# AndrewBoessen/3DGS

Measured on AMD Instinct MI355X. Metric: fwd+bwd iterations/s (one view per GPU), 1e6 gaussians @1920x1080, SH deg 3, higher is better.
Workload: dtype f32; 1 GPU; BASELINE configs[2]: synthetic 1000000 gaussians, 1920x1080, SH deg 3, forward+backward; parallelism=single GPU, exchange=none, backend=none, M=1000000, S=3499903, num_pairs=22157704, scene_seed=15717

## Files before the change

3dgs_amd/_lib.py:

```python
import ctypes
import os
import subprocess

_HERE = os.path.dirname(os.path.abspath(__file__))
_CSRC = os.path.join(_HERE, "csrc")
LIB_PATH = os.path.join(_HERE, "libgsplat_hip.so")
_lib = None


class GsplatError(RuntimeError):
    def __init__(self, code, text):
        super().__init__(f"gsplat error {code}: {text}")
        self.code = code


def build(force=False):
    import fcntl
    srcs = [os.path.join(_CSRC, f) for f in os.listdir(_CSRC) if f.endswith((".hip", ".h")) or f == "Makefile"]
    srcs.append(os.path.join(_CSRC, "host", "gs_dataset.cpp"))
    srcs.append(os.path.join(_HERE, "..", "include", "gsplat_hip.h"))

    def stale():
        return force or not os.path.exists(LIB_PATH) or any(
            os.path.getmtime(s) > os.path.getmtime(LIB_PATH) for s in srcs)
# ... 154 lines not shown
    "gsplat_gather_rows": (_I, [_I, _I, _P, _P, _P, _P]),
    "gsplat_sample_by_weight": (_I, [_P, _I, _I, ctypes.c_ulonglong, _P, _P, _P]),
    "gsplat_mcmc_relocate": (_I, [_I, _P, _P, _P, _F, _P]),
    "gsplat_mcmc_add_noise": (_I, [_I, _P, _P, _P, _P, _F, ctypes.c_ulonglong, _P]),
    "gsplat_mcmc_regularize": (_I, [_I, _P, _P, _P, _F, _F, _P, _P, _P]),
    "gsplat_compact_masked_array": (_I, [_P, _P, _I, _I, _P, ctypes.POINTER(_I), _P]),
    "gsplat_scatter_masked_array": (_I, [_P, _P, _I, _I, _P, _P]),
    "gsplat_context_create": (_I, [ctypes.POINTER(_P), _I, _I, _I]),
    "gsplat_context_destroy": (_I, [_P]),
    "gsplat_context_bytes": (_S, [_P]),
    "gsplat_rasterize_image": (_I, [_P, ctypes.POINTER(Gaussians), ctypes.POINTER(Camera),
                                    ctypes.POINTER(RasterConfig), _F, _I, ctypes.POINTER(ForwardView), _P]),
    "gsplat_backward_pass": (_I, [_P, ctypes.POINTER(Gaussians), ctypes.POINTER(Camera), _P, _F, _I,
                                  ctypes.POINTER(Gradients), _P]),
    "gsplat_backward_gaussians_adam": (_I, [_P, ctypes.POINTER(Gaussians), ctypes.POINTER(Camera), _I,
                                            ctypes.POINTER(AdamFused), ctypes.POINTER(Gradients), _P]),
    "gsplat_context_set_render_only": (_I, [_P, _I]),
    "gsplat_context_set_lean_forward": (_I, [_P, _I]),
    "gsplat_context_set_depth": (_I, [_P, _I]),
    "gsplat_context_depth_map": (_I, [_P, ctypes.POINTER(_P)]),
    "gsplat_backward_render_depth": (_I, [_P, _P, _P, _P, _F, _P, _P, _P, _P]),
    "gsplat_backward_pass_depth": (_I, [_P, ctypes.POINTER(Gaussians), ctypes.POINTER(Camera), _P, _P, _P, _F, _I,
                                        ctypes.POINTER(Gradients), _P]),
    "gsplat_context_set_depth_mode": (_I, [_P, _I, _I]),
    "gsplat_context_depth_moment_map": (_I, [_P, ctypes.POINTER(_P)]),
    "gsplat_backward_render_depth2": (_I, [_P, _P, _P, _P, _P, _F, _P, _P, _P, _P]),
    "gsplat_backward_pass_depth2": (_I, [_P, ctypes.POINTER(Gaussians), ctypes.POINTER(Camera), _P, _P, _P, _P, _F, _I,
                                         ctypes.POINTER(Gradients), _P]),
    "gsplat_distortion_loss": (_I, [_P, _P, _P, _I, _I, _F, _I, _P, _P, _P, _P, _P]),
    "gsplat_depth_prior_loss": (_I, [_P, _P, _I, _I, _F, _I, _P, _P, _P]),
    "gsplat_depth_to_normal": (_I, [_P, _P, _I, _I, _F, _F, _F, _F, _I, _F, _P, _P]),
    "gsplat_depth_to_normal_backward": (_I, [_P, _P, _I, _I, _F, _F, _F, _F, _I, _F, _P, _I, _P, _P, _P]),
    "gsplat_normal_prior_loss": (_I, [_P, _P, _I, _I, _F, _I, _P, _P, _P]),
    "gsplat_normal_smoothness_loss": (_I, [_P, _P, _I, _I, _F, _F, _I, _P, _P, _P]),
    "gsplat_backward_gaussians_camera": (_I, [_P, ctypes.POINTER(Gaussians), ctypes.POINTER(Camera), _I,
                                              ctypes.POINTER(Gradients), _P, _P, _P]),
    "gsplat_backward_pass_camera": (_I, [_P, ctypes.POINTER(Gaussians), ctypes.POINTER(Camera), _P, _P, _P, _F, _I,
                                         ctypes.POINTER(Gradients), _P, _P, _P]),
    "gsplat_context_accumulate_contributions": (_I, [_P, _I, _P, _P, _P, _P]),
    "gsplat_context_render_features": (_I, [_P, _I, _I, _P, _P, _P]),
    "gsplat_context_lift_features": (_I, [_P, _I, _I, _P, _P, _P]),
    "gsplat_context_features_backward": (_I, [_P, _I, _I, _P, _P, _P]),
    "gsplat_feature_ce_loss": (_I, [_P, _P, _I, _I, _I, _F, _I, _P, _P, _P]),
    "gsplat_feature_l1_loss": (_I, [_P, _P, _P, _I, _I, _I, _F, _I, _P, _P, _P]),
    "gsplat_feature_cosine_loss": (_I, [_P, _P, _P, _I, _I, _I, _F, _I, _P, _P, _P]),
    "gsplat_feature_adam_step": (_I, [_P, _I, _I, _P, _P, _P, _P, _F, _F, _F, _F, _F, _F, _P]),
    "gsplat_bilagrid_slice": (_I, [_P, _I, _I, _I, _P, _I, _I, _P, _P]),
    "gsplat_bilagrid_slice_backward": (_I, [_P, _I, _I, _I, _P, _P, _I, _I, _I, _P, _P, _P]),
    "gsplat_bilagrid_tv_loss": (_I, [_P, _I, _I, _I, _F, _I, _P, _P, _P]),
    "gsplat_vq_assign": (_I, [_P, _P, _I, _I, _I, _P, _P, _P]),
    "gsplat_vq_update": (_I, [_P, _P, _P, _I, _I, _I, _P, _P]),
    "gsplat_context_set_absgrad": (_I, [_P, _I]),
    "gsplat_context_set_compact_lists": (_I, [_P, _I]),
    "gsplat_context_absgrad_uv": (_I, [_P, _P, _P]),
    "gsplat_pack_absgrad_norm": (_I, [_P, _I, _P, _P]),
    "gsplat_context_set_antialiased": (_I, [_P, _I]),
    "gsplat_compute_conic_antialiased": (_I, [_P, _P, _P, _F, _F, _F, _F, _F, _I, _P, _P, _P, _P, _P]),
    "gsplat_compute_conic_antialiased_backward": (_I, [_P, _P, _P, _P, _P, _P, _I, _P, _P, _P]),
    "gsplat_compute_filter3d": (_I, [_P, _I, _P, _P, _P, _P, _I, _F, _P, _P]),
    "gsplat_filter3d_apply": (_I, [_P, _P, _P, _I, _P, _P, _P]),
    "gsplat_filter3d_apply_backward": (_I, [_P, _P, _P, _P, _I, _P, _I, _P, _I, _P]),
    "gsplat_context_set_filter3d": (_I, [_P, _P]),
    "gsplat_context_set_preprocess_split": (_I, [_P, _I]),
    "gsplat_context_get_counters": (_I, [_P, ctypes.POINTER(ctypes.c_longlong), _I]),
    "gsplat_context_set_timing": (_I, [_P, _I]),
    "gsplat_context_set_timing_stages": (_I, [_P, ctypes.c_uint]),
    "gsplat_context_get_timing": (_I, [_P, ctypes.POINTER(ctypes.c_double), ctypes.POINTER(ctypes.c_longlong), _I]),
    "gsplat_pack_gradients_global": (_I, [_P, ctypes.POINTER(Gradients), _I, _I, _P, _P]),
    "gsplat_packed_gradient_width": (_I, [_I]),
    "gsplat_factored_gradient_width": (_I, [_I]),
    "gsplat_pack_gradients_factored": (_I, [_P, ctypes.POINTER(Gradients), _I, _I, _I, _P, _P]),
    "gsplat_unpack_gradients_factored": (_I, [_P, _P, _P, _I, _I, _I, _P, _P]),
}


def load():
    global _lib
    if _lib is not None:
        return _lib
    path = os.environ.get("GSPLAT_LIB")
    if not path:
        if os.environ.get("GSPLAT_NO_BUILD") == "1":
            if not os.path.exists(LIB_PATH):
                raise OSError(f"{LIB_PATH} is missing and GSPLAT_NO_BUILD=1 forbids building it")
        else:
            try:
                build()
            except (OSError, subprocess.CalledProcessError) as e:
                if not os.path.exists(LIB_PATH):
                    raise
                import sys
                print(f"[3dgs_amd] WARNING: rebuilding libgsplat_hip.so failed ({e}); loading the EXISTING library, "
                      "which may be older than the sources (the ABI version is checked below)", file=sys.stderr, flush=True)
        path = LIB_PATH
    import torch
    lib = ctypes.CDLL(path)
    for name, (res, args) in SIGNATURES.items():
        fn = getattr(lib, name)
        fn.restype = res
        fn.argtypes = args
    got = lib.gsplat_abi_version()
    if got != ABI_VERSION:
        raise RuntimeError(f"libgsplat_hip.so reports ABI {got}, this binding expects {ABI_VERSION}: stale library")
    built_from, flags = lib.gsplat_source_hash().decode(), lib.gsplat_build_flags().decode()
    if built_from != source_hash() or flags:
        import sys
# ... 22 lines not shown
```

3dgs_amd/csrc/gs_context.h:

```cpp
#pragma once
#include "gs_common.h"
#include "gs_render.h"

namespace gs {

int pre_split_default();
bool pre_join_late();
bool no_tile_order();
bool no_compact_lists();
bool no_segments();
bool no_fwd_segments();
double fwd_segments_gate();

}

struct gsplat_context {
  int max_gaussians = 0, max_width = 0, max_height = 0;
  gs::DeviceBuffer mask, counters, rank, xyz_c_all, uv_all;
  gs::DeviceBuffer c2g, xyz_c, uv, sigma, conic, J, rgb, radius, recs, counts, offsets, grad_rows, hitmask;
  gs::DeviceBuffer keys_a, keys_b, pay_a, pay_b, sorted, temp, bin_table;
  gs::DeviceBuffer blockmasks;
  gs::DeviceBuffer ranges, image, T_px, n_px;
  gs::DeviceBuffer tile_tops, tile_order;
  bool order_ready = false;
  gs::DeviceBuffer ids_c, masks_c, n_c_px, tile_useful;
  bool compact_lists = true;
  bool compact_written = false;
  bool compact_ready = false;
  long long n_compact_backwards = 0;
  gs::DeviceBuffer seg_first, seg_extra, seg_chk;
  gs::DeviceBuffer fseg_first, fseg_blocks, fseg_gran, fseg_part, fseg_stop;
  bool depth = false;
  bool depth_ready = false;
  bool rows_depth = false;
  gs::DeviceBuffer depth_map, seg_chk_d, fseg_part_d;
  bool depth_inverse = false, depth_moment = false;
  bool depth_inverse_ready = false, depth_moment_ready = false;
  gs::DeviceBuffer depth2_map, seg_chk_q, fseg_part_q;
  bool absgrad = false;
  bool rows_abs = false;
  bool antialiased = false;
  bool fwd_antialiased = false;
  const float *filter3d = nullptr;
  const float *fwd_filter3d = nullptr;
  gs::DeviceBuffer f3d_scale, f3d_opacity;
  void *fseg_gran_zeroed = nullptr;
  size_t fseg_gran_zeroed_bytes = 0;
  unsigned int fseg_epoch = 0;
  int fseg_poll_budget = gs::kFwdPollBudget, fseg_thin_layer = gs::kFwdThinLayerDefault;
  double fseg_gate = -1.0;
  unsigned long long n_segmented_forwards = 0;
  gs::Figures fig;
  int seg_cap = 0;
  bool seg_ready = false;
  unsigned long long n_segmented_backwards = 0;
  const unsigned char *last_mask = nullptr;
  int *h_words = nullptr;
  bool dense_route = false;
  int forced_route = 0;
  bool rows_ready = false;
  bool backward_seen = false, rows_zeroed = false;
  bool render_only = false;
  bool lean = false;
  int pre_split = gs::pre_split_default();
  hipStream_t pre_side = nullptr;
  hipEvent_t ev_pre_fork = nullptr, ev_pre_join = nullptr;
  gs::DeviceBuffer chunk_first;
  gs::DeviceBuffer kept;
  gs::DeviceBuffer dir_grad;
  gs::DeviceBuffer cam_rows;
  gs::SortFork fork;
  volatile unsigned long long *h_pub = nullptr;
  unsigned long long *d_pub = nullptr, ticket = 0;
  unsigned long long *pair_counters() const { return counters.as<unsigned long long>(); }
  int *slice_counts() const { return counters.as<int>() + 128; }
  int *fseg_fallbacks() const { return counters.as<int>() + 128 + gs::kBinBlocks; }
  static constexpr int kStages = 8, kSlots = 32;
  unsigned int timing = 0;
  hipEvent_t ev[kSlots][2 * kStages] = {};
  unsigned char pending[kSlots][kStages] = {};
  double stage_ms[kStages] = {};
  long long stage_n[kStages] = {};
  long long fwd_calls = 0;
  long long n_forwards = 0, n_tail_redone = 0, n_compact_walks = 0, n_instance_growths = 0, n_ordered_backwards = 0;
  int slot = 0;
  void mark(int stage, bool stop, hipStream_t st) {
    if (!((timing >> stage) & 1u)) return;
    (void)hipEventRecord(ev[slot][2 * stage + (stop ? 1 : 0)], st);
    if (stop) pending[slot][stage] = 1;
  }
  void harvest(int sl) {
    for (int k = 0; k < kStages; ++k)
      if (pending[sl][k]) {
        float ms = 0.f;
        if (hipEventElapsedTime(&ms, ev[sl][2 * k], ev[sl][2 * k + 1]) == hipSuccess) { stage_ms[k] += ms; stage_n[k] += 1; }
        pending[sl][k] = 0;
      }
  }
  int N = 0, M = 0, l_max = 0, width = 0, height = 0;
  float tan_fovx = 0.f, tan_fovy = 0.f, mh_dist = 0.f;
  size_t S = 0;
  long long last_longest = -1;
  bool have_forward = false;
  bool lists_ready = false;
  enum : unsigned { kCounted = 1u, kOutput = 2u };
  template <class C, class F>
  static void each_buffer(C &c, F &&f) {
    constexpr unsigned W = kCounted, O = kCounted | kOutput;
    f(c.mask, O); f(c.uv_all, O); f(c.xyz_c_all, O); f(c.sigma, O); f(c.conic, O); f(c.J, O); f(c.rgb, O); f(c.radius, O);
    f(c.sorted, O); f(c.ranges, O); f(c.image, O); f(c.T_px, O); f(c.n_px, O);
    f(c.counters, W); f(c.rank, W); f(c.c2g, W); f(c.xyz_c, W); f(c.uv, W); f(c.recs, W); f(c.counts, W); f(c.offsets, W);
    f(c.grad_rows, W); f(c.hitmask, W); f(c.keys_a, W); f(c.keys_b, W); f(c.pay_a, W); f(c.pay_b, W); f(c.temp, W);
    f(c.bin_table, 0u);
    f(c.blockmasks, W); f(c.kept, W); f(c.tile_tops, W); f(c.tile_order, W);
    f(c.ids_c, W); f(c.masks_c, W); f(c.n_c_px, W); f(c.tile_useful, W);
    f(c.seg_first, W); f(c.seg_extra, W); f(c.seg_chk, W);
    f(c.fseg_first, W); f(c.fseg_blocks, W); f(c.fseg_gran, W); f(c.fseg_part, W); f(c.fseg_stop, W);
    f(c.dir_grad, W); f(c.cam_rows, W); f(c.depth_map, W); f(c.seg_chk_d, W); f(c.fseg_part_d, W);
    f(c.depth2_map, W); f(c.seg_chk_q, W); f(c.fseg_part_q, W);
    f(c.f3d_scale, W); f(c.f3d_opacity, W);
    f(c.chunk_first, 0u);
  }
  void forward_outputs(gs::DeviceBuffer *out[13]) {
    int n = 0;
    each_buffer(*this, [&](gs::DeviceBuffer &b, unsigned flags) { if (flags & kOutput) out[n++] = &b; });
  }
  size_t bytes() const {
    size_t total = 0;
    each_buffer(*this, [&](const gs::DeviceBuffer &b, unsigned flags) { if (flags & kCounted) total += b.bytes; });
    return total;
  }
  void release() {
    gs::pool_unwatch(&last_mask);
    last_mask = nullptr;
    each_buffer(*this, [](gs::DeviceBuffer &b, unsigned) { b.release(); });
    fseg_gran_zeroed = nullptr;
    fork.destroy();
    if (pre_side) { (void)hipStreamDestroy(pre_side); pre_side = nullptr; }
    if (ev_pre_fork) { (void)hipEventDestroy(ev_pre_fork); ev_pre_fork = nullptr; }
    if (ev_pre_join) { (void)hipEventDestroy(ev_pre_join); ev_pre_join = nullptr; }
    if (h_words) (void)hipHostFree(h_words);
    h_words = nullptr;
    if (h_pub) { (void)hipHostFree((void *)h_pub); h_pub = nullptr; d_pub = nullptr; }
    for (int a = 0; a < kSlots; ++a)
      for (int b = 0; b < 2 * kStages; ++b)
        if (ev[a][b]) { (void)hipEventDestroy(ev[a][b]); ev[a][b] = nullptr; }
  }
};

namespace gs {
size_t instance_room(const gsplat_context *c);
int reserve_instances(gsplat_context *c, size_t S, int num_tiles, hipStream_t st);
}
```

3dgs_amd/csrc/gs_context.hip:

```cpp
#include <cstdlib>
#include <new>
#include <vector>

#include "gs_context.h"
#include "gs_launch.h"

namespace gs {

static bool env_is(const char *name, char c) { const char *e = getenv(name); return e && e[0] == c; }
static int env_digit(const char *name, int lo, int hi, int otherwise) {
  const char *e = getenv(name);
  return e && e[0] >= '0' + lo && e[0] <= '0' + hi ? e[0] - '0' : otherwise;
}
static double env_number(const char *name, double otherwise) { const char *e = getenv(name); return e && e[0] ? atof(e) : otherwise; }

int pre_split_default() { static const int v = env_digit("GSPLAT_PRE_SPLIT", 0, 2, 0); return v; }
bool pre_join_late() { static const bool v = env_is("GSPLAT_PRE_JOIN", 'l'); return v; }
bool no_tile_order() { static const bool v = env_is("GSPLAT_NO_TILE_ORDER", '1'); return v; }
bool no_compact_lists() { static const bool v = env_is("GSPLAT_NO_COMPACT_LISTS", '1'); return v; }
bool no_segments() { static const bool v = env_is("GSPLAT_NO_SEGMENTS", '1'); return v; }
bool no_fwd_segments() { static const bool v = env_is("GSPLAT_NO_FWD_SEGMENTS", '1'); return v; }
double fwd_segments_gate() { static const double v = env_number("GSPLAT_FWD_SEGMENTS_GATE", 3.0); return v; }

size_t instance_room(const gsplat_context *c) {
  size_t room = c->keys_a.bytes / sizeof(unsigned int);
  room = std::min(room, c->keys_b.bytes / sizeof(unsigned int));
  room = std::min(room, c->pay_a.bytes / sizeof(unsigned long long));
  room = std::min(room, c->pay_b.bytes / sizeof(unsigned long long));
  room = std::min(room, c->sorted.bytes / sizeof(int));
  room = std::min(room, c->blockmasks.bytes / sizeof(unsigned short));
  room = std::min(room, c->ids_c.bytes / sizeof(int));
  room = std::min(room, c->masks_c.bytes / sizeof(unsigned short));
  return room;
}

int reserve_instances(gsplat_context *c, size_t S, int num_tiles, hipStream_t st) {
  int rc;
  const void *pay_before = c->pay_a.ptr, *sorted_before = c->sorted.ptr;
  if ((rc = c->keys_a.reserve((S + 1) * sizeof(unsigned int)))) return rc;
  if ((rc = c->keys_b.reserve((S + 1) * sizeof(unsigned int)))) return rc;
  if ((rc = c->pay_a.reserve((S + 1) * sizeof(unsigned long long)))) return rc;
  if ((rc = c->pay_b.reserve((S + 1) * sizeof(unsigned long long)))) return rc;
  if ((rc = c->sorted.reserve((S + 1) * sizeof(int)))) return rc;
  if (c->pay_a.ptr != pay_before) GS_HIP(hipMemsetAsync(c->pay_a.ptr, 0, c->pay_a.bytes, st));
  if (c->sorted.ptr != sorted_before) GS_HIP(hipMemsetAsync(c->sorted.ptr, 0, c->sorted.bytes, st));
  if ((rc = c->blockmasks.reserve((S + 1) * sizeof(unsigned short)))) return rc;
  if ((rc = c->ids_c.reserve((S + 1) * sizeof(int)))) return rc;
  if ((rc = c->masks_c.reserve((S + 1) * sizeof(unsigned short)))) return rc;
  if ((rc = c->temp.reserve(gs::binning_temp_bytes((size_t)c->max_gaussians, S ? S : 1, num_tiles)))) return rc;
  return GSPLAT_OK;
}

}

extern "C" {

int gsplat_context_create(gsplat_context **out, int max_gaussians, int max_width, int max_height) {
  GS_REQUIRE(out != nullptr, "out is null");
  GS_REQUIRE(max_gaussians > 0 && max_width > 0 && max_height > 0, "capacities must be positive");
  gsplat_context *c = new (std::nothrow) gsplat_context();
  GS_REQUIRE(c != nullptr, "out of host memory");
  c->max_gaussians = max_gaussians; c->max_width = max_width; c->max_height = max_height;
  const size_t N = (size_t)max_gaussians, P = (size_t)max_width * max_height;
  const size_t T = (size_t)((max_width + 15) / 16) * ((max_height + 15) / 16);
  int rc = GSPLAT_OK;
  {
    gs::DeviceBuffer *outs[13];
    c->forward_outputs(outs);
    for (gs::DeviceBuffer *b : outs) b->pooled = true;
  }
  auto R = [&](gs::DeviceBuffer &b, size_t bytes) { if (!rc) rc = b.reserve(bytes); };
  R(c->mask, N + 16); R(c->counters, 512 + gs::kBinBlocks * 4 + 64); R(c->rank, (N + 1) * 4); R(c->xyz_c_all, N * 12); R(c->uv_all, N * 8);
  R(c->c2g, N * 4); R(c->xyz_c, N * 12); R(c->uv, N * 8); R(c->sigma, N * 24); R(c->conic, N * 12); R(c->J, N * 24);
  R(c->rgb, N * 12); R(c->radius, N * 16); R(c->recs, N * 48); R(c->counts, (N + 1) * 4); R(c->offsets, (N + 1) * 4);
  R(c->grad_rows, N * 64); R(c->hitmask, N * 8);
// ... 52 lines not shown
  if (compact_to_global) *compact_to_global = have ? c->c2g.as<int>() : nullptr;
  if (num_gaussians) *num_gaussians = have ? c->N : 0;
  if (num_culled) *num_culled = have ? c->M : 0;
  return GSPLAT_OK;
}

int gsplat_context_detach_forward_outputs(gsplat_context *c) {
  GS_REQUIRE(c != nullptr, "null context");
  GS_REQUIRE(c->n_forwards > 0 && c->mask.ptr != nullptr, "no forward whose outputs could be handed over");
  GS_REQUIRE(!c->lean && !c->render_only, "a lean / render-only forward does not fill all ForwardPassData arrays");
  gs::DeviceBuffer *outs[13];
  c->forward_outputs(outs);
  for (gs::DeviceBuffer *b : outs) (void)b->detach();
  c->have_forward = false;
  c->lists_ready = false;
  c->rows_ready = false;
  return GSPLAT_OK;
}

int gsplat_context_set_depth(gsplat_context *c, int enabled) {
  GS_REQUIRE(c != nullptr, "null context");
  c->depth = enabled != 0;
  c->depth_inverse = c->depth_moment = false;
  return GSPLAT_OK;
}

int gsplat_context_set_depth_mode(gsplat_context *c, int inverse, int moment) {
  GS_REQUIRE(c != nullptr, "null context");
  c->depth = true;
  c->depth_inverse = inverse != 0;
  c->depth_moment = moment != 0;
  return GSPLAT_OK;
}

int gsplat_context_set_antialiased(gsplat_context *c, int enabled) {
  GS_REQUIRE(c != nullptr, "null context");
  c->antialiased = enabled != 0;
  return GSPLAT_OK;
}

int gsplat_context_set_filter3d(gsplat_context *c, const float *filter3d) {
  GS_REQUIRE(c != nullptr, "null context");
  if (filter3d) GS_REQUIRE_DEV(filter3d);
  c->filter3d = filter3d;
  return GSPLAT_OK;
}

int gsplat_context_set_compact_lists(gsplat_context *c, int enabled) {
  GS_REQUIRE(c != nullptr, "null context");
  c->compact_lists = enabled != 0;
  return GSPLAT_OK;
}

int gsplat_context_set_absgrad(gsplat_context *c, int enabled) {
  GS_REQUIRE(c != nullptr, "null context");
  c->absgrad = enabled != 0;
  return GSPLAT_OK;
}

int gsplat_context_accumulate_contributions(gsplat_context *c, int num_gaussians, float *weight_sum, float *weight_max,
                                            int *pixels, void *stream) {
  GS_REQUIRE(c != nullptr, "null context");
  GS_REQUIRE(weight_sum || weight_max || pixels, "no statistic asked for: weight_sum, weight_max and pixels are all NULL");
  GS_REQUIRE(c->lists_ready, "no forward pass recorded in this context");
  GS_REQUIRE(num_gaussians == c->N, "does not match the recorded forward");
  if (weight_sum) GS_REQUIRE_DEV(weight_sum);
  if (weight_max) GS_REQUIRE_DEV(weight_max);
  if (pixels) GS_REQUIRE_DEV(pixels);
  return gs::launch_contributions(c->recs.as<float4>(), c->sorted.as<int>(), c->ranges.as<int>(), c->n_px.as<int>(),
                                  c->c2g.as<int>(), c->width, c->height, weight_sum, weight_max, pixels,
                                  (hipStream_t)stream);
}

int gsplat_context_render_features(gsplat_context *c, int num_gaussians, int channels, const float *features, float *out,
                                   void *stream) {
  GS_REQUIRE(c != nullptr, "null context");
  GS_REQUIRE(c->lists_ready, "no forward pass recorded in this context");
  GS_REQUIRE(num_gaussians == c->N, "does not match the recorded forward");
  GS_REQUIRE(channels >= 1 && channels <= 512, "channels must be 1 .. 512");
  GS_REQUIRE_DEV(features);
  GS_REQUIRE_DEV(out);
  return gs::launch_features_fwd(c->recs.as<float4>(), c->sorted.as<int>(), c->ranges.as<int>(), c->n_px.as<int>(),
                                 c->c2g.as<int>(), c->width, c->height, channels, features, out, (hipStream_t)stream);
}

int gsplat_context_lift_features(gsplat_context *c, int num_gaussians, int channels, const float *map, float *lifted,
                                 void *stream) {
  GS_REQUIRE(c != nullptr, "null context");
  GS_REQUIRE(c->lists_ready, "no forward pass recorded in this context");
  GS_REQUIRE(num_gaussians == c->N, "does not match the recorded forward");
  GS_REQUIRE(channels >= 1 && channels <= 512, "channels must be 1 .. 512");
  GS_REQUIRE_DEV(map);
  GS_REQUIRE_DEV(lifted);
  return gs::launch_features_lift(c->recs.as<float4>(), c->sorted.as<int>(), c->ranges.as<int>(), c->n_px.as<int>(),
                                  c->c2g.as<int>(), c->width, c->height, channels, map, lifted, (hipStream_t)stream);
}

int gsplat_context_features_backward(gsplat_context *c, int num_gaussians, int channels, const float *features,
                                     const float *grad_map, void *stream) {
  GS_REQUIRE(c != nullptr, "null context");
  GS_REQUIRE(c->lists_ready, "no forward pass recorded in this context");
  GS_REQUIRE(c->have_forward && c->rows_ready,
             "gsplat_backward_render has not run for this forward pass: the feature term is added to its gradient rows");
  GS_REQUIRE(num_gaussians == c->N, "does not match the recorded forward");
  GS_REQUIRE(channels >= 1 && channels <= 512, "channels must be 1 .. 512");
  GS_REQUIRE(features != nullptr && gs::check_device_ptr(features, "features", __func__) == GSPLAT_OK,
// ... 22 lines not shown
  return GSPLAT_OK;
}

int gsplat_context_set_binning_route(gsplat_context *c, int route) {
  GS_REQUIRE(c != nullptr, "null context");
  GS_REQUIRE(route >= 0 && route <= 2, "route: 0 auto, 1 counting sort, 2 radix sorts");
  c->forced_route = route;
  return GSPLAT_OK;
}

int gsplat_context_set_segment_options(gsplat_context *c, int poll_budget, int thin_layer_blocks, float gate) {
  GS_REQUIRE(c != nullptr, "null context");
  if (poll_budget >= 0) c->fseg_poll_budget = poll_budget > 0 ? poll_budget : 1;
  if (thin_layer_blocks >= 0) c->fseg_thin_layer = thin_layer_blocks;
  if (gate >= 0.0f) c->fseg_gate = gate;
  return GSPLAT_OK;
}

int gsplat_context_set_timing_stages(gsplat_context *c, unsigned int stage_mask) {
  GS_REQUIRE(c != nullptr, "null context");
  if (stage_mask && !c->ev[0][0]) {
    for (int a = 0; a < gsplat_context::kSlots; ++a)
      for (int b = 0; b < 2 * gsplat_context::kStages; ++b) GS_HIP(hipEventCreate(&c->ev[a][b]));
  }
  GS_HIP(hipDeviceSynchronize());
  for (int a = 0; a < gsplat_context::kSlots; ++a) c->harvest(a);
  for (int k = 0; k < gsplat_context::kStages; ++k) { c->stage_ms[k] = 0; c->stage_n[k] = 0; }
  c->timing = stage_mask & ((1u << gsplat_context::kStages) - 1u);
  return GSPLAT_OK;
}

int gsplat_context_get_counters(gsplat_context *c, long long *out, int n) {
  GS_REQUIRE(c && out && n >= 0, "null argument");
  long long fmax = c->fig.max, fsum = c->fig.sum;
  unsigned int best = 0;
  for (int sl = 0; sl < 2; ++sl) {
    const unsigned long long w0 = __atomic_load_n(&c->h_pub[8 + 4 * sl], __ATOMIC_RELAXED);
    const unsigned long long w1 = __atomic_load_n(&c->h_pub[9 + 4 * sl], __ATOMIC_RELAXED);
    const unsigned int tag = (unsigned int)(w0 >> 32);
    if (tag != 0 && tag == (unsigned int)(w1 >> 32) && tag >= best && tag <= (unsigned int)(c->ticket & 0xFFFFFFFFull)) {
      best = tag; fmax = (long long)(int)(unsigned int)w0; fsum = (long long)(int)(unsigned int)w1;
    }
  }
  int fallbacks = 0;
  if (n > 9 && c->counters.ptr) GS_HIP(hipMemcpy(&fallbacks, c->fseg_fallbacks(), sizeof(int), hipMemcpyDeviceToHost));
  long long useful = 0;
  if (n > 11 && c->compact_written && c->have_forward) {
    const size_t tiles = (size_t)((c->width + 15) / 16) * ((c->height + 15) / 16);
    std::vector<int> h(tiles);
    GS_HIP(hipDeviceSynchronize());
    GS_HIP(hipMemcpy(h.data(), c->tile_useful.ptr, tiles * sizeof(int), hipMemcpyDeviceToHost));
    for (int u : h) useful += u;
  }
  const long long v[12] = {c->n_forwards, c->n_tail_redone, c->n_compact_walks, c->n_instance_growths, c->n_ordered_backwards,
                           (long long)c->n_segmented_backwards, (long long)c->n_segmented_forwards, fmax, fsum, fallbacks,
                           c->n_compact_backwards, useful};
  for (int k = 0; k < n && k < 12; ++k) out[k] = v[k];
  return 12;
}

int gsplat_context_set_render_only(gsplat_context *c, int enabled) {
  GS_REQUIRE(c != nullptr, "null context");
  c->render_only = enabled != 0;
  if (c->render_only) c->have_forward = false;
  return GSPLAT_OK;
}

int gsplat_context_set_preprocess_split(gsplat_context *c, int mode) {
  GS_REQUIRE(c != nullptr, "null context");
  GS_REQUIRE(mode >= 0 && mode <= 2, "mode: 0 one kernel, 1 two kernels in sequence, 2 two kernels side by side");
  c->pre_split = mode;
  return GSPLAT_OK;
}

int gsplat_context_set_lean_forward(gsplat_context *c, int enabled) {
  GS_REQUIRE(c != nullptr, "null context");
  c->lean = enabled != 0;
  return GSPLAT_OK;
}

int gsplat_context_set_timing(gsplat_context *c, int enabled) {
  return gsplat_context_set_timing_stages(c, enabled ? ~0u : 0u);
}

int gsplat_context_get_timing(gsplat_context *c, double *stage_ms_sum, long long *stage_count, int max_stages) {
  GS_REQUIRE(c && stage_ms_sum && stage_count, "null argument");
  GS_HIP(hipDeviceSynchronize());
  for (int a = 0; a < gsplat_context::kSlots; ++a) c->harvest(a);
  for (int k = 0; k < max_stages && k < gsplat_context::kStages; ++k) {
    stage_ms_sum[k] = c->stage_ms[k];
    stage_count[k] = c->stage_n[k];
  }
  return gsplat_context::kStages;
}

}
```

3dgs_amd/csrc/gs_fused.hip:

```cpp
#include <cmath>
#include <algorithm>

#include "gs_context.h"
#include "gs_launch.h"
#include "gs_pergaussian_args.h"

extern "C" {

struct FwdCall {
  const gsplat_gaussians *g; const gsplat_camera *cam; const gsplat_raster_config *cfg;
  float bg; hipStream_t st;
  int l_max, N, W, H, ntx, nty, num_tiles;
  float tan_fovx, tan_fovy;
  bool compact;
  bool beside;
  bool ro, mid;
  bool sparse, keys_ok;
  int *bin_table;
  unsigned long long ticket;
  gs::DepthMaps dmap;
  bool join_pending;
  bool segmented_this_forward;
};
static int check_forward_args(const gsplat_context *c, const gsplat_gaussians *g, const gsplat_camera *cam,
                              const gsplat_raster_config *cfg, int l_max) {
  static const char fn[] = "gsplat_rasterize_image";
  GS_REQUIRE_IN(fn, c && g && cam && cfg, "null argument struct");
  GS_REQUIRE_IN(fn, l_max >= 0 && l_max <= 3, "l_max must be 0..3");
  const int N = g->num_gaussians, W = cam->width, H = cam->height;
  GS_REQUIRE_IN(fn, N > 0, "num_gaussians must be positive");
  if (N > c->max_gaussians || W > c->max_width || H > c->max_height || W <= 0 || H <= 0) {
    gs::set_error("gsplat_rasterize_image: %d gaussians / %dx%d exceed the context capacity %d / %dx%d", N, W, H,
                  c->max_gaussians, c->max_width, c->max_height);
    return GSPLAT_ERR_CAPACITY;
  }
  GS_REQUIRE_DEV_IN(fn, g->xyz); GS_REQUIRE_DEV_IN(fn, g->rgb); GS_REQUIRE_DEV_IN(fn, g->opacity); GS_REQUIRE_DEV_IN(fn, g->scale);
  GS_REQUIRE_DEV_IN(fn, g->quaternion); GS_REQUIRE_DEV_IN(fn, cam->view); GS_REQUIRE_DEV_IN(fn, cam->proj);
  if (l_max > 0) GS_REQUIRE_DEV_IN(fn, g->sh);
  GS_REQUIRE_IN(fn, ((uintptr_t)g->quaternion & 15) == 0, "quaternion must be 16-byte aligned");
  GS_REQUIRE_IN(fn, !(c->antialiased && c->pre_split),
                "anti-aliased mode has no two-kernel forward (gsplat_context_set_preprocess_split / GSPLAT_PRE_SPLIT must be 0)");
  GS_REQUIRE_IN(fn, N <= (64 << 20), "more than 64 Mi gaussians: the cull's per-slice ballots would not fit its LDS");
  return GSPLAT_OK;
}

static int reclaim_outputs(gsplat_context *c, hipStream_t st) {
  c->have_forward = c->lists_ready = c->rows_ready = c->order_ready = c->depth_ready = c->rows_depth = c->rows_abs = false;
  c->depth_inverse_ready = c->depth_moment_ready = false;
  gs::pool_unwatch(&c->last_mask);
  c->last_mask = nullptr;
  gs::DeviceBuffer *outs[13];
  c->forward_outputs(outs);
  for (gs::DeviceBuffer *b : outs)
    if (b->ptr == nullptr) {
      const int r = b->reserve_again(st);
      if (r) return r;
      if (b == &c->sorted) GS_HIP(hipMemsetAsync(b->ptr, 0, b->bytes, st));
    }
  return GSPLAT_OK;
}

static int plan_forward_call(gsplat_context *c, const gsplat_gaussians *g, const gsplat_camera *cam,
                             const gsplat_raster_config *cfg, float bg_color, int l_max, hipStream_t st, FwdCall &f) {
  int rc = GSPLAT_OK;
  f = {}; f.g = g; f.cam = cam; f.cfg = cfg; f.bg = bg_color; f.l_max = l_max; f.st = st;
  f.N = g->num_gaussians; f.W = cam->width; f.H = cam->height;
  f.ntx = (f.W + 15) / 16; f.nty = (f.H + 15) / 16; f.num_tiles = f.ntx * f.nty;
  f.tan_fovx = (float)f.W / (2.0f * cam->focal_x); f.tan_fovy = (float)f.H / (2.0f * cam->focal_y);
  if (c->depth) {
    if ((rc = c->depth_map.reserve((size_t)f.W * f.H * sizeof(float), st))) return rc;
    f.dmap.xyz_c = c->xyz_c.as<float>(); f.dmap.depth = c->depth_map.as<float>();
    f.dmap.inverse = c->depth_inverse; f.dmap.moment = c->depth_moment;
    if (c->depth_moment) {
      if ((rc = c->depth2_map.reserve((size_t)f.W * f.H * sizeof(float), st))) return rc;
      f.dmap.depth2 = c->depth2_map.as<float>();
    }
  }
  f.compact = gs::compact_walk(c->N, c->M, f.N);
  if (f.compact && (rc = c->kept.reserve((size_t)c->max_gaussians * sizeof(int)))) return rc;
  f.beside = c->pre_split == 2 && l_max > 0;
  if (f.beside) {
    if ((rc = c->chunk_first.reserve(((size_t)gs::bin_chunks(c->max_gaussians) + gs::kBinThreads / 64 + 1) * sizeof(int)))) return rc;
    if (!c->pre_side) {
      int lo_prio = 0, hi_prio = 0;
      GS_HIP(hipDeviceGetStreamPriorityRange(&lo_prio, &hi_prio));
      GS_HIP(hipStreamCreateWithPriority(&c->pre_side, hipStreamNonBlocking, lo_prio));
      GS_HIP(hipEventCreateWithFlags(&c->ev_pre_fork, hipEventDisableTiming));
      GS_HIP(hipEventCreateWithFlags(&c->ev_pre_join, hipEventDisableTiming));
    }
  }
  f.ro = c->render_only; f.mid = !f.ro && !c->lean;
  const bool want_dense = c->forced_route == 2 || (c->forced_route == 0 && c->dense_route);
  f.sparse = !want_dense && gs::binning_supports_counting_sort(f.num_tiles);
  if (f.sparse) {
    if ((rc = c->bin_table.reserve(gs::binning_table_bytes(f.num_tiles)))) return rc;
    f.bin_table = c->bin_table.as<int>();
  }
  f.keys_ok = cfg->near_thresh >= 1e-30f; f.ticket = ++c->ticket;
  return GSPLAT_OK;
}

static int launch_cull(gsplat_context *c, const FwdCall &f) {
  c->mark(0, false, f.st);
  gs::CullArgs a = {};
  a.xyz = f.g->xyz; a.view = f.cam->view; a.proj = f.cam->proj;
  a.N = f.N; a.width = f.W; a.height = f.H;
  a.near_thresh = f.cfg->near_thresh; a.padding = f.cfg->cull_mask_padding;
  if (!c->lean) { a.xyz_c = c->xyz_c_all.as<float>(); a.uv = c->uv_all.as<float>(); }
  a.mask = c->mask.as<unsigned char>(); a.rank = c->rank.as<int>();
  a.slice_counts = c->slice_counts(); a.pair_counters = c->pair_counters();
  if (f.compact) a.kept = c->kept.as<int>();
  if (f.beside && !f.compact) a.chunk_first = c->chunk_first.as<int>();
  if (int rc = gs::launch_project_cull(a, f.st)) return rc;
  c->mark(0, true, f.st);
  return GSPLAT_OK;
}

static int launch_colour(gsplat_context *c, const FwdCall &f, hipStream_t cst) {
  if (f.l_max == 0) return GSPLAT_OK;
  gs::ShColourArgs a = {};
  a.g = *f.g;
  a.mask = c->mask.as<unsigned char>();
  a.slice_counts = c->slice_counts();
  if (f.compact) a.kept = c->kept.as<int>();
  else a.chunk_first = c->chunk_first.as<int>();
  for (int k = 0; k < 3; ++k) a.campos[k] = f.cam->campos[k];
  if (f.beside) {
    if (f.mid) a.rgb_out = c->rgb.as<float>();
    a.recs = c->recs.as<float4>();
  } else {
    a.rank = c->rank.as<int>();
    a.rgb_out = c->rgb.as<float>();
  }
  a.l_max = f.l_max; a.compact = f.compact;
  return gs::launch_sh_colour(a, cst);
}

static int launch_per_gaussian(gsplat_context *c, FwdCall &f) {
  hipStream_t st = f.st;
  int rc = GSPLAT_OK;
  c->mark(1, false, st);
  const bool mid = f.mid;
  gs::PreprocessArgs a = {};
  a.g = *f.g; a.view = f.cam->view; a.proj = f.cam->proj;
  a.mask = c->mask.as<unsigned char>(); a.rank = c->rank.as<int>();
  a.slice_counts = c->slice_counts(); a.kept = c->kept.as<int>();
  a.width = f.W; a.height = f.H; a.ntx = f.ntx; a.nty = f.nty;
  a.fx = f.cam->focal_x; a.fy = f.cam->focal_y; a.tan_fovx = f.tan_fovx; a.tan_fovy = f.tan_fovy;
  a.mh_dist = f.cfg->mh_dist;
  for (int k = 0; k < 3; ++k) a.campos[k] = f.cam->campos[k];
  a.c2g = c->c2g.as<int>(); a.xyz_c = c->xyz_c.as<float>(); a.uv = c->uv.as<float>();
  if (mid) { a.sigma = c->sigma.as<float>(); a.conic = c->conic.as<float>(); a.J = c->J.as<float>(); a.rgb = c->rgb.as<float>(); }
  a.radius = c->radius.as<float>(); a.recs = c->recs.as<float4>(); a.counts = c->counts.as<int>();
  a.hitmask = c->hitmask.as<unsigned long long>(); a.pairs = c->pair_counters();
  a.table = f.bin_table;
  a.l_max = f.l_max; a.store_mid = mid; a.compact = f.compact; a.antialiased = c->antialiased;
  if (c->pre_split) {
    const bool seq = f.l_max > 0 && c->pre_split == 1;
    if (seq) a.rgb = c->rgb.as<float>();
    hipStream_t cst = st;
    if (f.beside) {
      GS_HIP(hipEventRecord(c->ev_pre_fork, st));
      GS_HIP(hipStreamWaitEvent(c->pre_side, c->ev_pre_fork, 0));
      cst = c->pre_side;
    }
    if (seq && (rc = launch_colour(c, f, cst))) return rc;
    if ((rc = gs::launch_preprocess_geom(a, f.l_max == 0 ? 0 : f.beside ? 2 : 1, st))) return rc;
    if (f.beside) {
      if ((rc = launch_colour(c, f, cst))) return rc;
      GS_HIP(hipEventRecord(c->ev_pre_join, c->pre_side));
      if (gs::pre_join_late()) f.join_pending = true;
      else GS_HIP(hipStreamWaitEvent(st, c->ev_pre_join, 0));
    }
  } else if ((rc = gs::launch_preprocess(a, st))) {
    return rc;
  }
  c->fwd_antialiased = c->antialiased;
  return GSPLAT_OK;
}

static int queue_counts(gsplat_context *c, const FwdCall &f, size_t &room) {
  const int N = f.N; hipStream_t st = f.st;
  int rc = GSPLAT_OK;
  if (f.sparse) {
    if (gs::instance_room(c) < 2 && (rc = gs::reserve_instances(c, 4 * (size_t)N, f.num_tiles, st))) return rc;
    room = gs::instance_room(c) - 1;
    c->mark(1, true, st);
    c->mark(2, false, st);
    return gs::binning_offsets(f.ntx, f.nty, f.bin_table, c->keys_a.as<int>(), st);
  }
  rc = gs::scan_counts(N, c->counts.as<int>(), c->offsets.as<int>(), c->temp.ptr, c->temp.bytes, st);
  if (rc) return rc;
  c->mark(1, true, st);
  if ((rc = gs::launch_publish_counts(c->rank.as<int>() + N, c->offsets.as<int>() + N, c->pair_counters(), c->d_pub, f.ticket, st)))
    return rc;
  if (gs::instance_room(c) < 2 && (rc = gs::reserve_instances(c, 4 * (size_t)N, f.num_tiles, st))) return rc;
  room = gs::instance_room(c) - 1;
  c->mark(2, false, st);
  return gs::launch_tile_emit(c->uv.as<float>(), c->xyz_c.as<float>(), c->radius.as<float>(), f.ntx, f.nty, N,
                              c->mask.as<unsigned char>(), c->rank.as<int>(), c->offsets.as<int>(),
                              c->hitmask.as<unsigned long long>(), (long long)room, c->keys_a.as<unsigned int>(),
                              c->pay_a.as<unsigned long long>(), st);
}

static gs::TileSegments backward_segments(gsplat_context *c, int extra_cap) {
  gs::TileSegments seg = {};
  seg.granted = c->seg_first.as<int>();
  seg.extra = c->seg_extra.as<int2>();
  seg.extra_count = reinterpret_cast<int *>(seg.extra + extra_cap);
  seg.chk = c->seg_chk.as<float4>();
  seg.image = c->image.as<float>();
  seg.extra_cap = extra_cap;
  return seg;
}
static gs::RenderFwdArgs packed_forward_args(gsplat_context *c, const FwdCall &f, long long zero_vec) {
  gs::RenderFwdArgs a = {};
  a.recs = c->recs.as<float4>();
  a.sorted = c->sorted.as<int>();
  a.ranges = c->ranges.as<int>();
  a.width = f.W; a.height = f.H; a.bg = f.bg;
  a.n_out = c->n_px.as<int>();
  a.T_out = c->T_px.as<float>();
  a.image = c->image.as<float>();
  if (c->rows_zeroed) a.zero = c->grad_rows.as<float4>();
  a.zero_vec = zero_vec;
  if (!f.ro) a.masks_out = c->blockmasks.as<unsigned short>();
  a.depth = f.dmap;
  return a;
// ... 125 lines not shown
    if ((polls & 255) == 0) {
      const hipError_t q = hipStreamQuery(f.st);
      if (q != hipSuccess && q != hipErrorNotReady) {
        gs::set_error("gsplat_rasterize_image: %s while waiting for the counts", hipGetErrorString(q));
        return GSPLAT_ERR_HIP;
      }
      if ((drained = q == hipSuccess)) continue;
    }
    __builtin_ia32_pause();
  }
  __atomic_thread_fence(__ATOMIC_ACQUIRE);
  rec = gs::decode_record(w);
  if (!f.sparse) rec.longest = -1;
  if (rec.M == 0) {
    gs::set_error("gsplat_rasterize_image: no gaussians in view");
    return GSPLAT_ERR_NO_VISIBLE;
  }
  return GSPLAT_OK;
}

static int finish_radix_route(gsplat_context *c, const FwdCall &f, const gs::ForwardRecord &rec, size_t inst_cap) {
  const size_t S = rec.S; hipStream_t st = f.st;
  int rc = gs::reserve_instances(c, S, f.num_tiles, st);
  if (rc) return rc;
  if (S + 1 > gs::instance_room(c)) {
    gs::set_error("gsplat_rasterize_image: internal: %zu instances sorted in room for %zu", S, gs::instance_room(c));
    return GSPLAT_ERR_CAPACITY;
  }
  rc = gs::emit_sort_ranges(c->uv.as<float>(), c->xyz_c.as<float>(), c->radius.as<float>(), f.ntx, f.nty, f.N,
                            c->mask.as<unsigned char>(), c->rank.as<int>(), c->offsets.as<int>(), S,
                            c->keys_a.as<unsigned int>(), c->keys_b.as<unsigned int>(),
                            c->pay_a.as<unsigned long long>(), c->pay_b.as<unsigned long long>(),
                            c->sorted.as<int>(), c->ranges.as<int>(), c->temp.ptr, c->temp.bytes, st, S <= inst_cap,
                            c->hitmask.as<unsigned long long>());
  if (rc) return rc;
  c->mark(2, true, st);
  c->mark(4, false, st);
  if (f.join_pending) GS_HIP(hipStreamWaitEvent(st, c->ev_pre_join, 0));
  if ((rc = gs::launch_render_fwd(packed_forward_args(c, f, (long long)rec.M * 4), st))) return rc;
  c->compact_written = false;
  c->seg_ready = false;
  c->mark(4, true, st);
  c->order_ready = false;
  return GSPLAT_OK;
}

static void record_forward(gsplat_context *c, const FwdCall &f, const gs::ForwardRecord &rec, gsplat_forward_view *out) {
  if (f.segmented_this_forward) c->n_segmented_forwards++;
  c->N = f.N; c->M = rec.M; c->S = rec.S; c->l_max = f.l_max; c->width = f.W; c->height = f.H;
  c->last_mask = c->mask.as<unsigned char>();
  gs::pool_watch(c->last_mask, &c->last_mask);
  c->tan_fovx = f.tan_fovx; c->tan_fovy = f.tan_fovy; c->mh_dist = f.cfg->mh_dist;
  c->have_forward = !f.ro;
  c->lists_ready = true;
  c->depth_ready = c->depth;
  c->depth_inverse_ready = c->depth && f.dmap.inverse;
  c->depth_moment_ready = c->depth && f.dmap.moment;
  if (!out) return;
  const bool mid = f.mid;
  out->num_culled = (size_t)rec.M; out->num_pairs = (size_t)rec.pairs; out->num_splats = rec.S;
  out->mask = c->mask.as<unsigned char>(); out->compact_to_global = c->c2g.as<int>();
  out->uv = c->lean ? nullptr : c->uv_all.as<float>(); out->xyz_c = c->lean ? nullptr : c->xyz_c_all.as<float>();
  out->sigma = mid ? c->sigma.as<float>() : nullptr; out->conic = mid ? c->conic.as<float>() : nullptr;
  out->J = mid ? c->J.as<float>() : nullptr; out->precomputed_rgb = mid ? c->rgb.as<float>() : nullptr;
  out->radius = c->radius.as<float>(); out->uv_selected = c->uv.as<float>(); out->xyz_c_selected = c->xyz_c.as<float>();
  out->sorted_gaussians = c->sorted.as<int>(); out->splat_start_end_idx_by_tile_idx = c->ranges.as<int>();
  out->image = c->image.as<float>(); out->weight_per_pixel = c->T_px.as<float>();
  out->splats_per_pixel = c->n_px.as<int>();
}

int gsplat_rasterize_image(gsplat_context *c, const gsplat_gaussians *g, const gsplat_camera *cam,
                           const gsplat_raster_config *cfg, float bg_color, int l_max, gsplat_forward_view *out,
                           void *stream) {
  int rc = check_forward_args(c, g, cam, cfg, l_max);
  if (rc) return rc;
  hipStream_t st = (hipStream_t)stream;
  if ((rc = reclaim_outputs(c, st))) return rc;
  gsplat_gaussians filtered;
  if (c->filter3d) {
    GS_REQUIRE_DEV(c->filter3d);
    if ((rc = c->f3d_scale.reserve((size_t)c->max_gaussians * 3 * sizeof(float), st))) return rc;
    if ((rc = c->f3d_opacity.reserve((size_t)c->max_gaussians * sizeof(float), st))) return rc;
    if ((rc = gs::launch_filter3d_apply(g->scale, g->opacity, c->filter3d, g->num_gaussians, c->f3d_scale.as<float>(),
                                        c->f3d_opacity.as<float>(), st))) return rc;
    filtered = *g; filtered.scale = c->f3d_scale.as<float>(); filtered.opacity = c->f3d_opacity.as<float>();
    g = &filtered;
  }
  c->fwd_filter3d = c->filter3d;
  FwdCall f;
  if ((rc = plan_forward_call(c, g, cam, cfg, bg_color, l_max, st, f))) return rc;
  if (c->timing) {
    c->slot = (int)(c->fwd_calls % gsplat_context::kSlots);
    c->harvest(c->slot);
  }
  c->fwd_calls++;
  if ((rc = launch_cull(c, f))) return rc;
  if ((rc = launch_per_gaussian(c, f))) return rc;
  size_t room = 0;
  if ((rc = queue_counts(c, f, room))) return rc;
  if (c->rows_zeroed) c->backward_seen = false;
  c->rows_zeroed = c->backward_seen && !f.ro;
  const long long spec_hint = f.sparse ? gs::speculative_longest(c->last_longest) : -1;
  if (f.sparse && (rc = queue_sparse_tail(c, f, room, spec_hint, true))) return rc;
  gs::ForwardRecord rec;
  if ((rc = wait_for_record(c, f, rec))) return rc;
  c->dense_route = gs::binning_next_route_is_radix(f.sparse, rec.S, f.num_tiles, rec.longest);
  c->last_longest = rec.longest;
  c->n_forwards++;
  if (f.compact) c->n_compact_walks++;
  if (!f.sparse) {
    if ((rc = finish_radix_route(c, f, rec, room))) return rc;
  } else if (gs::tail_needs_redo(rec.S, room, spec_hint, rec.longest, f.keys_ok)) {
    c->n_tail_redone++;
    if (rec.S > room) {
      c->n_instance_growths++;
      if ((rc = gs::reserve_instances(c, rec.S + rec.S / 4, f.num_tiles, st))) return rc;
    }
    GS_HIP(hipMemsetAsync(c->keys_a.ptr, 0, sizeof(int), st));
    if ((rc = queue_sparse_tail(c, f, rec.S, rec.longest, false))) return rc;
  }
  c->compact_ready = c->compact_written && rec.longest >= 0 && rec.longest <= gs::kSegSplitMin;
  record_forward(c, f, rec, out);
  return GSPLAT_OK;
}

int gsplat_backward_render(gsplat_context *c, const float *grad_image, float bg_color, float *rgb_global,
                           void *stream) {
  return gsplat_backward_render_split(c, grad_image, bg_color, rgb_global, nullptr, nullptr, stream);
}

int gsplat_backward_render_split(gsplat_context *c, const float *grad_image, float bg_color, float *rgb_global,
                                 float *common, float *uv_norm, void *stream) {
  return gsplat_backward_render_depth2(c, grad_image, nullptr, nullptr, nullptr, bg_color, rgb_global, common, uv_norm, stream);
}

int gsplat_backward_render_depth(gsplat_context *c, const float *grad_image, const float *grad_depth,
                                 const float *grad_alpha, float bg_color, float *rgb_global, float *common, float *uv_norm,
                                 void *stream) {
  return gsplat_backward_render_depth2(c, grad_image, grad_depth, grad_alpha, nullptr, bg_color, rgb_global, common, uv_norm, stream);
}

int gsplat_backward_render_depth2(gsplat_context *c, const float *grad_image, const float *grad_depth,
                                  const float *grad_alpha, const float *grad_depth2, float bg_color, float *rgb_global,
                                  float *common, float *uv_norm, void *stream) {
  GS_REQUIRE(c != nullptr, "null context");
  GS_REQUIRE(c->have_forward, "no forward pass recorded in this context");
  GS_REQUIRE_DEV(grad_image);
  if (rgb_global) GS_REQUIRE_DEV(rgb_global);
  if (common) {
    GS_REQUIRE(rgb_global != nullptr, "the common rows are cleared by the pass that scatters g_rgb: rgb_global is needed");
    GS_REQUIRE_DEV(common);
    GS_REQUIRE(((uintptr_t)common & 15) == 0, "common must be 16-byte aligned");
  }
  if (uv_norm) { GS_REQUIRE(common != nullptr, "uv_norm goes with common"); GS_REQUIRE_DEV(uv_norm); }
  const bool depth = grad_depth != nullptr || grad_alpha != nullptr || grad_depth2 != nullptr;
  if (grad_depth) GS_REQUIRE_DEV(grad_depth);
  if (grad_alpha) GS_REQUIRE_DEV(grad_alpha);
  if (grad_depth2) GS_REQUIRE_DEV(grad_depth2);
  GS_REQUIRE(!depth || c->depth_ready, "depth / alpha gradients need a forward that rendered depth (gsplat_context_set_depth)");
  GS_REQUIRE(!grad_depth2 || c->depth_moment_ready,
             "grad_depth2 needs a forward that rendered the second moment (gsplat_context_set_depth_mode)");
  GS_REQUIRE(!(depth && c->depth_moment_ready && c->absgrad),
             "the moment option has no absgrad form: depth gradients of such a forward cannot be taken in absgrad mode");
  hipStream_t st = (hipStream_t)stream;
  const int M = c->M, W = c->width, H = c->height;
  c->rows_ready = false;
// ... 96 lines not shown
  }
  if (!out) out = &kNoArrays;
  const bool leaves = !common && !(adam && (out == &kNoArrays || adam_mode == 1)) && !(cam_grad && out == &kNoArrays);
  return check_gradient_arrays(fn, out, l_max, leaves);
}

static int backward_gaussians_impl(const char *fn, gsplat_context *c, const gsplat_gaussians *g, const gsplat_camera *cam,
                                   int l_max, const gsplat_gradients *out, float *common, float *uv_norm, int first_gaussian,
                                   int end_gaussian, void *stream, const gsplat_adam_fused *adam = nullptr, int adam_mode = 2,
                                   float *adam_dir = nullptr, float *grad_view = nullptr, float *grad_campos = nullptr) {
  int rc = check_backward_gaussians(fn, c, g, cam, l_max, out, common, first_gaussian, end_gaussian, adam != nullptr,
                                    adam_mode, grad_view, grad_campos);
  if (rc) return rc;
  const bool cam_grad = grad_view != nullptr;
  if (!out) out = &kNoArrays;
  hipStream_t st = (hipStream_t)stream;
  const float *raw_scale = g->scale, *raw_opacity = g->opacity;
  gsplat_gaussians filtered;
  if (c->fwd_filter3d) {
    filtered = *g; filtered.scale = c->f3d_scale.as<float>(); filtered.opacity = c->f3d_opacity.as<float>();
    g = &filtered;
  }
  const int M = c->M, W = c->width, H = c->height;
  const float fx = cam->focal_x, fy = cam->focal_y;
  const float fov_x = (float)(2.0 * atan((double)W / (2.0 * (double)fx)));
  const float fov_y = (float)(2.0 * atan((double)H / (2.0 * (double)fy)));
  const float tan_fovx = tanf(fov_x * 0.5f), tan_fovy = tanf(fov_y * 0.5f);
  const bool whole = first_gaussian == 0 && end_gaussian == g->num_gaussians;
  const int span = whole ? M : std::min(M, end_gaussian - first_gaussian);
  const int n_cam_rows = gs::div_up(span, 64);
  if (cam_grad && span > 0 && (rc = c->cam_rows.reserve((size_t)n_cam_rows * 16 * sizeof(double), st))) return rc;
  if (span == 0) {
    if (cam_grad) {
      GS_HIP(hipMemsetAsync(grad_view, 0, 12 * sizeof(float), st));
      GS_HIP(hipMemsetAsync(grad_campos, 0, 3 * sizeof(float), st));
    }
    return GSPLAT_OK;
  }
  c->mark(7, false, st);
  gs::PreprocessBwdArgs a = {};
  a.g = *g; a.view = cam->view; a.proj = cam->proj;
  a.M = M; a.c2g = c->c2g.as<int>(); a.xyz_c = c->xyz_c.as<float>(); a.rows = c->grad_rows.as<float4>();
  a.fx = fx; a.fy = fy; a.tan_fovx = tan_fovx; a.tan_fovy = tan_fovy;
  a.fwd_tan_fovx = c->tan_fovx; a.fwd_tan_fovy = c->tan_fovy;
  a.mh_dist = c->mh_dist;
  for (int k = 0; k < 3; ++k) a.campos[k] = cam->campos[k];
  a.width = W; a.height = H;
  a.out = *out; a.common = common; a.uv_norm = uv_norm;
  a.ranged = whole ? 0 : 1; a.first = first_gaussian; a.end = end_gaussian; a.span = span;
  if (adam) { a.adam = adam; a.adam_mode = adam_mode; a.adam_dir = adam_dir; }
  if (cam_grad) { a.cam_rows = c->cam_rows.as<double>(); a.grad_view = grad_view; a.grad_campos = grad_campos; }
  a.l_max = l_max; a.rows_depth = c->rows_depth; a.rows_abs = c->rows_abs;
  a.antialiased = c->fwd_antialiased;
  if ((rc = gs::launch_preprocess_bwd(a, st))) return rc;
  if (c->fwd_filter3d) {
    const int lo = whole ? 0 : first_gaussian, hi = whole ? 0 : end_gaussian;
    if (common)
      rc = gs::launch_filter3d_apply_bwd(raw_scale, raw_opacity, c->fwd_filter3d, c->c2g.as<int>(), M, common + 4, 12,
                                         common + 3, 12, true, lo, hi, span, st);
    else if (out->grad_scale && out->grad_opacity)
      rc = gs::launch_filter3d_apply_bwd(raw_scale, raw_opacity, c->fwd_filter3d, c->c2g.as<int>(), M, out->grad_scale, 3,
                                         out->grad_opacity, 1, false, lo, hi, span, st);
    if (rc) return rc;
  }
  c->mark(7, true, st);
  return GSPLAT_OK;
}

int gsplat_backward_gaussians(gsplat_context *c, const gsplat_gaussians *g, const gsplat_camera *cam, int l_max,
                              const gsplat_gradients *out, void *stream) {
  GS_REQUIRE(out != nullptr, "null argument struct");
  return backward_gaussians_impl(__func__, c, g, cam, l_max, out, nullptr, nullptr, 0, g ? g->num_gaussians : 0, stream);
}

int gsplat_backward_gaussians_range(gsplat_context *c, const gsplat_gaussians *g, const gsplat_camera *cam, int l_max,
                                    const gsplat_gradients *out, int first_gaussian, int end_gaussian, void *stream) {
  GS_REQUIRE(out != nullptr, "null argument struct");
  return backward_gaussians_impl(__func__, c, g, cam, l_max, out, nullptr, nullptr, first_gaussian, end_gaussian, stream);
}

int gsplat_backward_gaussians_split(gsplat_context *c, const gsplat_gaussians *g, const gsplat_camera *cam, int l_max,
                                    float *common, float *uv_norm, int first_gaussian, int end_gaussian, void *stream) {
  GS_REQUIRE_DEV(common);
  GS_REQUIRE(((uintptr_t)common & 15) == 0, "common must be 16-byte aligned");
  if (uv_norm) GS_REQUIRE_DEV(uv_norm);
  return backward_gaussians_impl(__func__, c, g, cam, l_max, nullptr, common, uv_norm, first_gaussian, end_gaussian, stream);
}

int gsplat_backward_gaussians_adam(gsplat_context *c, const gsplat_gaussians *g, const gsplat_camera *cam, int l_max,
                                   const gsplat_adam_fused *opt, const gsplat_gradients *out, void *stream) {
  GS_REQUIRE(opt != nullptr && g != nullptr, "null argument struct");
  for (int k = 0; k < 6; ++k) {
    if (k == 2 && l_max == 0) continue;
    GS_REQUIRE_DEV(opt->exp_avg[k]); GS_REQUIRE_DEV(opt->exp_avg_sq[k]);
  }
  GS_REQUIRE(((uintptr_t)opt->exp_avg[5] & 15) == 0 && ((uintptr_t)opt->exp_avg_sq[5] & 15) == 0,
             "the quaternion moments must be 16-byte aligned");
  if (opt->uv_grad_accum) GS_REQUIRE_DEV(opt->uv_grad_accum);
  if (opt->grad_accum_dur) GS_REQUIRE_DEV(opt->grad_accum_dur);
  GS_REQUIRE(opt->mode >= 0 && opt->mode <= 2,
             "mode: 0 all six groups in one kernel, 1 SH and position left to the optimizer kernels, 2 the SH group in a kernel of its own in front");
  if (opt->mode == 1) {
    GS_REQUIRE(out != nullptr, "mode 1 hands grad_xyz and grad_precompute_rgb to the optimizer kernels: `out` is needed");
    GS_REQUIRE_DEV(out->grad_xyz);
    if (l_max > 0) GS_REQUIRE_DEV(out->grad_precompute_rgb);
  }
// ... 73 lines not shown
```

3dgs_amd/csrc/gs_math.h:

```cpp
#pragma once
#include <hip/hip_runtime.h>
#include <math.h>

namespace gs {

struct Mat34 { float m[12]; };
struct Mat44 { float m[16]; };

__device__ __forceinline__ Mat34 load_view(const float *__restrict__ view) {
  Mat34 v;
#pragma unroll
  for (int k = 0; k < 12; ++k) v.m[k] = view[k];
  return v;
}
__device__ __forceinline__ Mat44 load_proj(const float *__restrict__ proj) {
  Mat44 p;
#pragma unroll
  for (int k = 0; k < 16; ++k) p.m[k] = proj[k];
  return p;
}

__device__ __forceinline__ int f2i_sat(float v) {
  if (v != v) return 0;
  if (v >= 2147483647.0f) return 2147483647;
// ... 86 lines not shown
  o.m[5] = J[3] * w02 + J[4] * w12 + J[5] * w22;
  o.v[0] = s[0] * o.m[0] + s[1] * o.m[1] + s[2] * o.m[2];
  o.v[1] = s[0] * o.m[3] + s[1] * o.m[4] + s[2] * o.m[5];
  o.v[2] = s[1] * o.m[0] + s[3] * o.m[1] + s[4] * o.m[2];
  o.v[3] = s[1] * o.m[3] + s[3] * o.m[4] + s[4] * o.m[5];
  o.v[4] = s[2] * o.m[0] + s[4] * o.m[1] + s[5] * o.m[2];
  o.v[5] = s[2] * o.m[3] + s[4] * o.m[4] + s[5] * o.m[5];
  return o;
}

template <bool kRho = false>
__device__ __forceinline__ void conic_radius(const float *J, const float *s, const Mat34 &vw, float mh_dist,
                                             float *conic , float *radius , float *rho = nullptr,
                                             float *cov = nullptr ) {
  const MV a = mv_from(J, s, vw);
  const float raw00 = a.m[0] * a.v[0] + a.m[1] * a.v[2] + a.m[2] * a.v[4];
  const float cov01 = a.m[0] * a.v[1] + a.m[1] * a.v[3] + a.m[2] * a.v[5];
  const float raw11 = a.m[3] * a.v[1] + a.m[4] * a.v[3] + a.m[5] * a.v[5];
  const float cov00 = raw00 + 0.3f;
  const float cov11 = raw11 + 0.3f;
  const float det = cov00 * cov11 - cov01 * cov01;
  if constexpr (kRho) {
    const float det0 = raw00 * raw11 - cov01 * cov01;
    *rho = sqrtf(fmaxf(0.0f, det0 / det));
    cov[0] = raw00; cov[1] = cov01; cov[2] = raw11;
  }
  const float inv_det = 1.0f / det;
  conic[0] = cov11 * inv_det;
  conic[1] = -cov01 * inv_det;
  conic[2] = cov00 * inv_det;
  const float mid = 0.5f * (cov00 + cov11);
  const float lambda_term = sqrtf(fmaxf(0.1f, mid * mid - det));
  const float lambda1 = mid + lambda_term, lambda2 = mid - lambda_term;
  radius[0] = ceilf(mh_dist * sqrtf(lambda1));
  radius[1] = ceilf(mh_dist * sqrtf(lambda2));
  const float th = 0.5f * atan2f(2.0f * cov01, cov00 - cov11);
  float sn, cs;
  sincosf(th, &sn, &cs);
  radius[2] = sn;
  radius[3] = cs;
}

#define GS_SH_C0 0.28209479177387814f
#define GS_SH_C1 0.4886025119029199f
#define GS_SH_C2 1.0925484305920792f
#define GS_SH_C3 0.31539156525252005f
#define GS_SH_C4 0.5462742152960396f
#define GS_SH_C5 0.5900435899266435f
#define GS_SH_C6 2.890611442640554f
#define GS_SH_C7 0.4570457994644658f
#define GS_SH_C8 0.3731763325901154f
#define GS_SH_C9 1.445305721320277f

template <int L>
__device__ __forceinline__ void sh_basis(float x, float y, float z, float *Y) {
  Y[0] = GS_SH_C0;
  if constexpr (L >= 1) {
    Y[1] = GS_SH_C1 * y; Y[2] = GS_SH_C1 * z; Y[3] = GS_SH_C1 * x;
  }
  if constexpr (L >= 2) {
    const float xx = x * x, yy = y * y, zz = z * z;
    Y[4] = GS_SH_C2 * (x * y);
    Y[5] = GS_SH_C2 * (y * z);
    Y[6] = GS_SH_C3 * (2.0f * zz - xx - yy);
    Y[7] = GS_SH_C2 * (x * z);
    Y[8] = GS_SH_C4 * (xx - yy);
    if constexpr (L >= 3) {
      Y[9] = GS_SH_C5 * (y * (3.0f * xx - yy));
      Y[10] = GS_SH_C6 * (x * y * z);
      Y[11] = GS_SH_C7 * (y * (4.0f * zz - xx - yy));
      Y[12] = GS_SH_C8 * (z * (2.0f * zz - 3.0f * xx - 3.0f * yy));
      Y[13] = GS_SH_C7 * (x * (4.0f * zz - xx - yy));
      Y[14] = GS_SH_C9 * (z * (xx - yy));
      Y[15] = GS_SH_C5 * (x * (xx - 3.0f * yy));
    }
  }
}

template <int L>
__device__ __forceinline__ void sh_basis_grad(float x, float y, float z, float (*d)[3]) {
  d[0][0] = d[0][1] = d[0][2] = 0.0f;
  if constexpr (L >= 1) {
    d[1][0] = 0; d[1][1] = GS_SH_C1; d[1][2] = 0;
    d[2][0] = 0; d[2][1] = 0; d[2][2] = GS_SH_C1;
    d[3][0] = GS_SH_C1; d[3][1] = 0; d[3][2] = 0;
  }
  if constexpr (L >= 2) {
    const float xx = x * x, yy = y * y, zz = z * z;
    d[4][0] = GS_SH_C2 * y; d[4][1] = GS_SH_C2 * x; d[4][2] = 0;
    d[5][0] = 0; d[5][1] = GS_SH_C2 * z; d[5][2] = GS_SH_C2 * y;
    d[6][0] = GS_SH_C3 * (-2.0f * x); d[6][1] = GS_SH_C3 * (-2.0f * y); d[6][2] = GS_SH_C3 * (4.0f * z);
    d[7][0] = GS_SH_C2 * z; d[7][1] = 0; d[7][2] = GS_SH_C2 * x;
    d[8][0] = GS_SH_C4 * (2.0f * x); d[8][1] = GS_SH_C4 * (-2.0f * y); d[8][2] = 0;
    if constexpr (L >= 3) {
      d[9][0] = GS_SH_C5 * (6.0f * x * y); d[9][1] = GS_SH_C5 * (3.0f * xx - 3.0f * yy); d[9][2] = 0;
      d[10][0] = GS_SH_C6 * (y * z); d[10][1] = GS_SH_C6 * (x * z); d[10][2] = GS_SH_C6 * (x * y);
      d[11][0] = GS_SH_C7 * (-2.0f * x * y); d[11][1] = GS_SH_C7 * (4.0f * zz - xx - 3.0f * yy);
      d[11][2] = GS_SH_C7 * (8.0f * y * z);
      d[12][0] = GS_SH_C8 * (-6.0f * x * z); d[12][1] = GS_SH_C8 * (-6.0f * y * z);
      d[12][2] = GS_SH_C8 * (6.0f * zz - 3.0f * xx - 3.0f * yy);
      d[13][0] = GS_SH_C7 * (4.0f * zz - 3.0f * xx - yy); d[13][1] = GS_SH_C7 * (-2.0f * x * y);
      d[13][2] = GS_SH_C7 * (8.0f * x * z);
      d[14][0] = GS_SH_C9 * (2.0f * x * z); d[14][1] = GS_SH_C9 * (-2.0f * y * z); d[14][2] = GS_SH_C9 * (xx - yy);
      d[15][0] = GS_SH_C5 * (3.0f * xx - 3.0f * yy); d[15][1] = GS_SH_C5 * (-6.0f * x * y); d[15][2] = 0;
    }
  }
}

__device__ __forceinline__ void view_dir(float px, float py, float pz, float cx, float cy, float cz, float &dx,
                                         float &dy, float &dz, float &len) {
  const float fx = px - cx, fy = py - cy, fz = pz - cz;
  len = sqrtf(fx * fx + fy * fy + fz * fz) + 1e-9f;
  dx = fx / len; dy = fy / len; dz = fz / len;
}

template <int L>
__device__ __forceinline__ void sh_to_rgb(const float *__restrict__ sh, const float *__restrict__ band0, float dx,
                                          float dy, float dz, float *rgb) {
  constexpr int n = (L + 1) * (L + 1);
  float Y[n];
  sh_basis<L>(dx, dy, dz, Y);
  float r = band0[0] * Y[0] + 0.5f, g = band0[1] * Y[0] + 0.5f, b = band0[2] * Y[0] + 0.5f;
#pragma unroll
  for (int k = 0; k < n - 1; ++k) {
    r += sh[3 * k + 0] * Y[k + 1];
    g += sh[3 * k + 1] * Y[k + 1];
    b += sh[3 * k + 2] * Y[k + 1];
  }
  rgb[0] = r; rgb[1] = g; rgb[2] = b;
}

struct TileRect { int x0, x1, y0, y1; };

__device__ __forceinline__ TileRect coarse_rect(float u, float v, float r_major, int ntx, int nty) {
  const int radius_tiles = f2i_sat(ceilf(r_major * 0.0625f)) + 1;
  const int ptx = f2i_sat(floorf(u / 16.0f));
  const int pty = f2i_sat(floorf(v / 16.0f));
  long long sx = (long long)ptx - radius_tiles, ex = (long long)ptx + radius_tiles + 1;
  long long sy = (long long)pty - radius_tiles, ey = (long long)pty + radius_tiles + 1;
  if (sx < 0) sx = 0;
  if (ex > ntx) ex = ntx;
  if (sy < 0) sy = 0;
  if (ey > nty) ey = nty;
  if (ex < sx) ex = sx;
  if (ey < sy) ey = sy;
  TileRect r;
  r.x0 = (int)sx; r.x1 = (int)ex; r.y0 = (int)sy; r.y1 = (int)ey;
  return r;
}

struct Obb {
  float c[8];
  float mnx, mxx, mny, mxy;
  float a2x, a2y, mn2, mx2;
  float a3x, a3y, mn3, mx3;
};

__device__ __forceinline__ Obb make_obb(float u, float v, float r_major, float r_minor, float sin_t, float cos_t) {
  Obb o;
// ... 182 lines not shown
  dJ[0] = dm00 * w00 + dm01 * w01 + dm02 * w02;
  dJ[1] = dm00 * w10 + dm01 * w11 + dm02 * w12;
  dJ[2] = dm00 * w20 + dm01 * w21 + dm02 * w22;
  dJ[3] = dm10 * w00 + dm11 * w01 + dm12 * w02;
  dJ[4] = dm10 * w10 + dm11 * w11 + dm12 * w12;
  dJ[5] = dm10 * w20 + dm11 * w21 + dm12 * w22;
}

__device__ __forceinline__ void sigma_bwd(const RotScale &rs, const float *g , float *dQ, float *dSc) {
  const float *Rm = rs.R;
  const float Sx = rs.s[0], Sy = rs.s[1], Sz = rs.s[2];
  const float w = rs.q[0], x = rs.q[1], y = rs.q[2], z = rs.q[3];
  float M[9];
  M[0] = Rm[0] * Sx; M[1] = Rm[1] * Sy; M[2] = Rm[2] * Sz;
  M[3] = Rm[3] * Sx; M[4] = Rm[4] * Sy; M[5] = Rm[5] * Sz;
  M[6] = Rm[6] * Sx; M[7] = Rm[7] * Sy; M[8] = Rm[8] * Sz;
  float dSg[9];
  dSg[0] = g[0]; dSg[1] = 0.5f * g[1]; dSg[2] = 0.5f * g[2];
  dSg[3] = 0.5f * g[1]; dSg[4] = g[3]; dSg[5] = 0.5f * g[4];
  dSg[6] = 0.5f * g[2]; dSg[7] = 0.5f * g[4]; dSg[8] = g[5];
  float dM[9], dR[9];
#pragma unroll
  for (int r = 0; r < 3; ++r)
#pragma unroll
    for (int c = 0; c < 3; ++c)
      dM[3 * r + c] = 2.0f * (dSg[3 * r] * M[c] + dSg[3 * r + 1] * M[3 + c] + dSg[3 * r + 2] * M[6 + c]);
  dR[0] = dM[0] * Sx; dR[1] = dM[1] * Sy; dR[2] = dM[2] * Sz;
  dR[3] = dM[3] * Sx; dR[4] = dM[4] * Sy; dR[5] = dM[5] * Sz;
  dR[6] = dM[6] * Sx; dR[7] = dM[7] * Sy; dR[8] = dM[8] * Sz;
  const float dsx = Rm[0] * dM[0] + Rm[3] * dM[3] + Rm[6] * dM[6];
  const float dsy = Rm[1] * dM[1] + Rm[4] * dM[4] + Rm[7] * dM[7];
  const float dsz = Rm[2] * dM[2] + Rm[5] * dM[5] + Rm[8] * dM[8];
  dSc[0] = dsx * Sx; dSc[1] = dsy * Sy; dSc[2] = dsz * Sz;
  float dw = 0.0f, dx = 0.0f, dy = 0.0f, dz = 0.0f;
  dw += dR[1] * (-2.0f * z) + dR[2] * (2.0f * y);
  dx += dR[1] * (2.0f * y) + dR[2] * (2.0f * z);
  dy += dR[0] * (-4.0f * y) + dR[1] * (2.0f * x) + dR[2] * (2.0f * w);
  dz += dR[0] * (-4.0f * z) + dR[1] * (-2.0f * w) + dR[2] * (2.0f * x);
  dw += dR[3] * (2.0f * z) + dR[5] * (-2.0f * x);
  dx += dR[3] * (2.0f * y) + dR[4] * (-4.0f * x) + dR[5] * (-2.0f * w);
  dy += dR[3] * (2.0f * x) + dR[5] * (2.0f * z);
  dz += dR[3] * (2.0f * w) + dR[4] * (-4.0f * z) + dR[5] * (2.0f * y);
  dw += dR[6] * (-2.0f * y) + dR[7] * (2.0f * x);
  dx += dR[6] * (2.0f * z) + dR[7] * (2.0f * w) + dR[8] * (-4.0f * x);
  dy += dR[6] * (-2.0f * w) + dR[7] * (2.0f * z) + dR[8] * (-4.0f * y);
  dz += dR[6] * (2.0f * x) + dR[7] * (2.0f * y);
  const float dot = w * dw + x * dx + y * dy + z * dz;
  dQ[0] = rs.inv_norm * (dw - dot * w);
  dQ[1] = rs.inv_norm * (dx - dot * x);
  dQ[2] = rs.inv_norm * (dy - dot * y);
  dQ[3] = rs.inv_norm * (dz - dot * z);
}

template <int L, bool kStoreGrad = true>
__device__ __forceinline__ void sh_bwd(const float *sh, const float *__restrict__ band0, float px,
                                       float py, float pz, float cx, float cy, float cz, const float *gr,
                                       float *sh_grad, float *__restrict__ band0_grad, float &ox,
                                       float &oy, float &oz) {
  constexpr int n = (L + 1) * (L + 1);
  float ux, uy, uz, len;
  view_dir(px, py, pz, cx, cy, cz, ux, uy, uz, len);
  float Y[n];
  float dY[n][3];
  sh_basis<L>(ux, uy, uz, Y);
  sh_basis_grad<L>(ux, uy, uz, dY);
  band0_grad[0] = gr[0] * Y[0]; band0_grad[1] = gr[1] * Y[0]; band0_grad[2] = gr[2] * Y[0];
  float dRx = 0, dGx = 0, dBx = 0, dRy = 0, dGy = 0, dBy = 0, dRz = 0, dGz = 0, dBz = 0;
  {
    const float R0 = band0[0], G0 = band0[1], B0 = band0[2];
    dRx += dY[0][0] * R0; dGx += dY[0][0] * G0; dBx += dY[0][0] * B0;
    dRy += dY[0][1] * R0; dGy += dY[0][1] * G0; dBy += dY[0][1] * B0;
    dRz += dY[0][2] * R0; dGz += dY[0][2] * G0; dBz += dY[0][2] * B0;
  }
#pragma unroll
  for (int k = 0; k < n - 1; ++k) {
    const float yv = Y[k + 1];
    const float Ri = sh[3 * k], Gi = sh[3 * k + 1], Bi = sh[3 * k + 2];
    if constexpr (kStoreGrad) { sh_grad[3 * k] = gr[0] * yv; sh_grad[3 * k + 1] = gr[1] * yv; sh_grad[3 * k + 2] = gr[2] * yv; }
    const float ddx = dY[k + 1][0], ddy = dY[k + 1][1], ddz = dY[k + 1][2];
    dRx += ddx * Ri; dGx += ddx * Gi; dBx += ddx * Bi;
    dRy += ddy * Ri; dGy += ddy * Gi; dBy += ddy * Bi;
    dRz += ddz * Ri; dGz += ddz * Gi; dBz += ddz * Bi;
  }
  const float tx = gr[0] * dRx + gr[1] * dGx + gr[2] * dBx;
  const float ty = gr[0] * dRy + gr[1] * dGy + gr[2] * dBy;
  const float tz = gr[0] * dRz + gr[1] * dGz + gr[2] * dBz;
  const float dot = tx * ux + ty * uy + tz * uz;
  ox = (tx - dot * ux) / len;
  oy = (ty - dot * uy) / len;
  oz = (tz - dot * uz) / len;
}

__device__ __forceinline__ void adam_values(float &p, float &m, float &v, float g, float lr, float b1, float b2, float eps,
                                            float bias1, float bias2) {
  if (g != g) g = 0.0f;
  const float mi = b1 * m + (1.0f - b1) * g;
  const float vi = b2 * v + (1.0f - b2) * g * g;
  const float m_hat = mi / bias1, v_hat = vi / bias2;
  p += -lr * m_hat / (sqrtf(v_hat) + eps);
  m = mi;
  v = vi;
}

}
```

3dgs_amd/csrc/gs_pergaussian_args.h:

```cpp
#pragma once
#include "gs_common.h"

namespace gs {

struct CullArgs {
  const float *xyz, *view, *proj;
  int N, width, height;
  float near_thresh;
  int padding;
  float *xyz_c, *uv;
  unsigned char *mask;
  int *rank, *slice_counts;
  unsigned long long *pair_counters;
  int *kept;
  int *chunk_first;
};

struct PreprocessArgs {
  gsplat_gaussians g;
  const float *view, *proj;
  const unsigned char *mask;
  int *rank;
  const int *slice_counts, *kept;
  int width, height, ntx, nty;
  float fx, fy, tan_fovx, tan_fovy, mh_dist, campos[3];
  int *c2g;
  float *xyz_c, *uv, *sigma, *conic, *J, *rgb, *radius;
  float4 *recs;
  int *counts;
  unsigned long long *hitmask, *pairs;
  int *table;
  int l_max;
  bool store_mid;
  bool compact;
  bool antialiased;
};

struct ShColourArgs {
  gsplat_gaussians g;
  const unsigned char *mask;
  const int *rank, *chunk_first, *slice_counts, *kept;
  float campos[3];
  float *rgb_out;
  float4 *recs;
  int l_max;
  bool compact;
};

struct PreprocessBwdArgs {
  gsplat_gaussians g;
  const float *view, *proj;
  int M;
  const int *c2g;
  const float *xyz_c;
  const float4 *rows;
  float fx, fy, tan_fovx, tan_fovy, fwd_tan_fovx, fwd_tan_fovy, mh_dist, campos[3];
  int width, height;
  gsplat_gradients out;
  float *common, *uv_norm;
  int ranged, first, end;
  int span;
  const gsplat_adam_fused *adam;
  float *adam_dir;
  double *cam_rows;
  float *grad_view, *grad_campos;
  int l_max;
  int adam_mode;
  bool rows_depth, rows_abs, antialiased;
};

struct ShAdamDirArgs {
  int M;
  const int *c2g;
  float *sh, *m, *v;
  float lr, b1, b2, eps, bias1, bias2;
  const float *xyz, *band0;
  float campos[3];
  const float4 *rows;
  float *dir_out;
  int l_max;
};

}
```

3dgs_amd/csrc/gs_preprocess.hip:

```cpp
#include <cstring>
#include <rocprim/rocprim.hpp>

#include "gs_common.h"
#include "gs_launch.h"
#include "gs_math.h"
#include "gs_pergaussian_args.h"
#include "gs_render.h"
#include "gs_rows.h"

namespace {

constexpr int kBlock = 256;

__global__ __launch_bounds__(gs::kBinThreads) void project_cull_kernel(const float *__restrict__ xyz,
                                                                       const float *__restrict__ view,
                                                                       const float *__restrict__ proj, int N, int width,
                                                                       int height, float near_thresh, int padding,
                                                                       float *__restrict__ xyz_c, float *__restrict__ uv,
                                                                       unsigned char *__restrict__ mask,
                                                                       int *__restrict__ rank,
                                                                       int *__restrict__ slice_counts,
                                                                       unsigned long long *__restrict__ pair_counters,
                                                                       int *__restrict__ kept,
                                                                       int *__restrict__ chunk_first) {
// ... 27 lines not shown
  }
  __syncthreads();
  if (w == 0) {
    const int n = trips * kWaves, per = (n + 63) / 64;
    int sum = 0;
    for (int e = lane * per; e < min(lane * per + per, n); ++e) sum += __popcll(s_ballot[e]);
    int incl = sum;
#pragma unroll
    for (int off = 1; off < 64; off <<= 1) {
      const int u = __shfl_up(incl, off, 64);
      if (lane >= off) incl += u;
    }
    int run = incl - sum;
    for (int e = lane * per; e < min(lane * per + per, n); ++e) { s_before[e] = run; run += __popcll(s_ballot[e]); }
    if (lane == 63) slice_counts[blockIdx.x] = incl;
  }
  __syncthreads();
  for (int t = 0; t < trips; ++t) {
    const int i = lo + t * gs::kBinThreads + (int)threadIdx.x;
    if (i < hi) {
      const unsigned long long bal = s_ballot[t * kWaves + w];
      const int r = s_before[t * kWaves + w] + __popcll(bal & ((1ull << lane) - 1ull));
      rank[i] = r;
      if (chunk_first && lane == 0) chunk_first[(lo >> 6) + t * kWaves + w] = s_before[t * kWaves + w];
      if (kept && ((bal >> lane) & 1ull)) kept[lo + r] = i;
    }
  }
}

template <int K>
__device__ __forceinline__ void wave_rows_store(float *__restrict__ dst, int j0, int p, int nact, const float *v, float *wsh) {
#pragma unroll
  for (int k = 0; k < K; ++k) wsh[p * K + k] = v[k];
  __builtin_amdgcn_fence(__ATOMIC_RELEASE, "wavefront");
  __builtin_amdgcn_wave_barrier();
  const int total = nact * K;
  float *out = dst + (size_t)j0 * K;
  for (int e = p * 4; e + 3 < total; e += nact * 4)
    *reinterpret_cast<gs::f4u *>(out + e) = __builtin_bit_cast(gs::f4u, *reinterpret_cast<const float4 *>(wsh + e));
  for (int e = (total & ~3) + p; e < total; e += nact) out[e] = wsh[e];
  __builtin_amdgcn_fence(__ATOMIC_ACQUIRE, "wavefront");
  __builtin_amdgcn_wave_barrier();
}

constexpr int kCoopTiles = 64;

struct PreOut {
  int *c2g;
  float *xyz_c, *uv, *sigma, *conic, *J, *rgb, *radius;
  float4 *recs;
  int *counts;
  unsigned long long *hitmask;
  unsigned long long *pairs;
};

template <int L, bool kStoreMid, bool kCompact, bool kAntialias = false>
__global__ __launch_bounds__(gs::kBinThreads) void preprocess_kernel(gsplat_gaussians g, const float *__restrict__ view,
                                                            const unsigned char *__restrict__ mask,
                                                            int *__restrict__ rank,
                                                            const int *__restrict__ slice_counts,
                                                            const int *__restrict__ kept,
                                                            const float *__restrict__ proj, int width, int height,
                                                            float fx, float fy,
                                                            float tan_fovx, float tan_fovy, float mh_dist, float cx,
                                                            float cy, float cz, int ntx, int nty, PreOut o,
                                                            int *__restrict__ table) {
  extern __shared__ int s_hist[];
  __shared__ int s_base[gs::kBinBlocks + 1];
  __shared__ int s_wsum[4];
  const int N = g.num_gaussians, T = ntx * nty;
  static_assert(gs::kBinBlocks == 256, "the scan below is written for four waves of slice counts");
  {
    const int lane = threadIdx.x & 63, w = threadIdx.x >> 6;
    int cnt = 0, incl = 0;
    if (threadIdx.x < gs::kBinBlocks) {
      cnt = slice_counts[threadIdx.x];
      incl = cnt;
#pragma unroll
      for (int off = 1; off < 64; off <<= 1) {
        const int u = __shfl_up(incl, off, 64);
        if (lane >= off) incl += u;
      }
      if (lane == 63) s_wsum[w] = incl;
    }
    if (table)
      for (int t = threadIdx.x; t < T; t += gs::kBinThreads) s_hist[t] = 0;
    __syncthreads();
    if (threadIdx.x < gs::kBinBlocks) {
      int before = 0;
      for (int q = 0; q < w; ++q) before += s_wsum[q];
      s_base[threadIdx.x] = before + incl - cnt;
      if (threadIdx.x == gs::kBinBlocks - 1) s_base[gs::kBinBlocks] = before + incl;
    }
    __syncthreads();
  }
  const int M = s_base[gs::kBinBlocks];
  const int C = gs::bin_chunks(N);
  unsigned long long coarse = 0;
  const int lane = threadIdx.x & 63;
  for (long long i = (long long)M + (long long)blockIdx.x * gs::kBinThreads + threadIdx.x; i <= N;
       i += (long long)gs::kBinBlocks * gs::kBinThreads)
    o.counts[i] = 0;
  if (blockIdx.x == 0 && threadIdx.x == 0) rank[N] = M;
  const int walk_chunks = gs::bin_chunks(kCompact ? M : N);
  for (int c = (int)blockIdx.x + gs::kBinBlocks * (int)(threadIdx.x >> 6); c < walk_chunks;
       c += gs::kBinBlocks * (gs::kBinThreads / 64)) {
  const int e = c * gs::kBinChunk + lane;
  int i = e, j = e;
  bool act;
  if constexpr (kCompact) {
    act = e < M;
    int sl = 0;
#pragma unroll
    for (int step = gs::kBinBlocks / 2; step > 0; step >>= 1) sl += (s_base[sl + step] <= e) ? step : 0;
    i = act ? kept[gs::kBinChunk * gs::bin_slice_first_chunk(C, sl) + (e - s_base[sl])] : 0;
    if (act) rank[i] = j;
  } else {
    const int sl = gs::bin_slice_of_chunk(C, c);
    if (i < N) {
      j = s_base[sl] + rank[i];
      rank[i] = j;
    }
    act = i < N && mask[i];
  }
  int hits = 0, span_n = 0;
  unsigned long long hm = 0ull;
  float bu = 0.0f, bv = 0.0f, br0 = 0.0f, br1 = 0.0f, br2 = 0.0f, br3 = 0.0f;
  if (act) {
    constexpr int n = (L + 1) * (L + 1);
    const gs::Mat34 vw = gs::load_view(view);
    float dx, dy, dz, len, rgb[3];
    gs::view_dir(g.xyz[3 * i], g.xyz[3 * i + 1], g.xyz[3 * i + 2], cx, cy, cz, dx, dy, dz, len);
    gs::sh_to_rgb<L>(g.sh + (size_t)i * (n - 1) * 3, g.rgb + 3 * i, dx, dy, dz, rgb);
    const float4 q = reinterpret_cast<const float4 *>(g.quaternion)[i];
    const gs::RotScale rs = gs::rot_scale(q.x, q.y, q.z, q.w, g.scale[3 * i], g.scale[3 * i + 1], g.scale[3 * i + 2]);
    float sg[6], J[6], con[3], rad[4];
    gs::sigma_from(rs, sg);
    __shared__ __attribute__((aligned(16))) float s_stage[kStoreMid ? gs::kBinThreads / 64 : 1][kStoreMid ? 64 * 12 : 4];
    int pp = 0, nact = 0, j0 = 0;
    float *wsh = s_stage[0];
    if constexpr (kStoreMid) {
      const unsigned long long actm = __ballot(true);
      nact = __popcll(actm);
      pp = __popcll(actm & ((1ull << lane) - 1ull));
      j0 = __builtin_amdgcn_readfirstlane(j - pp);
      wsh = s_stage[threadIdx.x >> 6];
      wave_rows_store<6>(o.sigma, j0, pp, nact, sg, wsh);
      wave_rows_store<3>(o.rgb, j0, pp, nact, rgb, wsh);
    }
    float x, y, z, u, v;
    {
      int i2 = i;
      asm volatile("" : "+v"(i2));
      gs::camera_space(vw, g.xyz[3 * i2], g.xyz[3 * i2 + 1], g.xyz[3 * i2 + 2], x, y, z);
      gs::to_screen(gs::load_proj(proj), x, y, z, width, height, u, v);
    }
    gs::jacobian(x, y, z, fx, fy, tan_fovx, tan_fovy, J);
    [[maybe_unused]] float rho = 1.0f, cov_raw[3];
    if constexpr (kAntialias) gs::conic_radius<true>(J, sg, vw, mh_dist, con, rad, &rho, cov_raw);
    else gs::conic_radius(J, sg, vw, mh_dist, con, rad);
    o.c2g[j] = i;
    o.uv[2 * j] = u; o.uv[2 * j + 1] = v;
    reinterpret_cast<float4 *>(o.radius)[j] = make_float4(rad[0], rad[1], rad[2], rad[3]);
    gs::SplatRec rec;
    if constexpr (kAntialias)
      rec = gs::make_record_opa(u, v, con[0], con[1], con[2], gs::sigmoid_fast(g.opacity[i]) * rho, rgb[0], rgb[1], rgb[2]);
    else
      rec = gs::make_record(u, v, con[0], con[1], con[2], g.opacity[i], rgb[0], rgb[1], rgb[2]);
    if constexpr (kStoreMid) {
      const float xyzc[3] = {x, y, z};
      wave_rows_store<3>(o.xyz_c, j0, pp, nact, xyzc, wsh);
      wave_rows_store<6>(o.J, j0, pp, nact, J, wsh);
      wave_rows_store<3>(o.conic, j0, pp, nact, con, wsh);
      const float rr[12] = {rec.r0.x, rec.r0.y, rec.r0.z, rec.r0.w, rec.r1.x, rec.r1.y, rec.r1.z, rec.r1.w,
                            rec.r2.x, rec.r2.y, rec.r2.z, rec.r2.w};
      wave_rows_store<12>(reinterpret_cast<float *>(o.recs), j0, pp, nact, rr, wsh);
    } else {
      o.xyz_c[3 * j] = x; o.xyz_c[3 * j + 1] = y; o.xyz_c[3 * j + 2] = z;
      o.recs[3 * j] = rec.r0; o.recs[3 * j + 1] = rec.r1; o.recs[3 * j + 2] = rec.r2;
    }
    bu = u; bv = v; br0 = rad[0]; br1 = rad[1]; br2 = rad[2]; br3 = rad[3];
  }
  if (act) {
    const gs::TileRect r = gs::coarse_rect(bu, bv, br0, ntx, nty);
    if (r.x1 > r.x0 && r.y1 > r.y0) {
      coarse += (unsigned long long)(r.x1 - r.x0) * (unsigned long long)(r.y1 - r.y0);
// ... 362 lines not shown
      bool h = false;
      if (p < total) {
        const int tx = sp.x0 + p / sh, ty = sp.y0 + p % sh;
        h = gs::obb_hits_tile(ob, tx, ty);
        if (h && table) atomicAdd(&s_hist[ty * ntx + tx], 1);
      }
      found += __popcll(__ballot(h));
    }
    if (lane == owner) hits = found;
  }
  late_act = act; late_j = j; late_hits = hits; late_hm = hm;
  }
  if (late_act) {
    o.counts[late_j] = late_hits;
    o.hitmask[late_j] = late_hm;
  }
#pragma unroll
  for (int off = 32; off > 0; off >>= 1) coarse += __shfl_down(coarse, off, 64);
  if ((threadIdx.x & 63) == 0 && coarse) atomicAdd(&o.pairs[(blockIdx.x * 16 + (threadIdx.x >> 6)) & 63], coarse);
  if (table) {
    __syncthreads();
    for (int t = threadIdx.x; t < T; t += gs::kBinThreads) table[(size_t)blockIdx.x * T + t] = s_hist[t];
  }
}

__global__ __launch_bounds__(64) void publish_counts_kernel(const int *__restrict__ rank_total,
                                                            const int *__restrict__ offsets_total,
                                                            const unsigned long long *__restrict__ pair_counters,
                                                            volatile unsigned long long *out,
                                                            unsigned long long ticket) {
  unsigned long long v = pair_counters[threadIdx.x];
#pragma unroll
  for (int off = 32; off > 0; off >>= 1) v += __shfl_down(v, off, 64);
  if (threadIdx.x == 0)
    gs::publish_record(out, ticket, (unsigned int)*rank_total, (unsigned int)*offsets_total, v, 0u);
}

}

namespace gs {

int launch_project_cull(const CullArgs &a, hipStream_t st) {
  const size_t slice_max = ((size_t)bin_chunks(a.N) / kBinBlocks + 2) * kBinChunk;
  const size_t trips = (slice_max + kBinThreads - 1) / kBinThreads + 1;
  project_cull_kernel<<<kBinBlocks, kBinThreads, trips * (kBinThreads / 64) * 12, st>>>(
      a.xyz, a.view, a.proj, a.N, a.width, a.height, a.near_thresh, a.padding, a.xyz_c, a.uv, a.mask, a.rank,
      a.slice_counts, a.pair_counters, a.kept, a.chunk_first);
  GS_LAUNCH_CHECK();
  return GSPLAT_OK;
}

template <class Kernel>
static void launch_per_gaussian(Kernel kernel, const PreprocessArgs &a, hipStream_t st) {
  const PreOut o = {a.c2g, a.xyz_c, a.uv, a.sigma, a.conic, a.J, a.rgb, a.radius, a.recs, a.counts, a.hitmask, a.pairs};
  const size_t hist_bytes = a.table ? (size_t)a.ntx * a.nty * sizeof(int) : 0;
  kernel<<<kBinBlocks, kBinThreads, hist_bytes, st>>>(a.g, a.view, a.mask, a.rank, a.slice_counts, a.kept, a.proj, a.width,
                                                      a.height, a.fx, a.fy, a.tan_fovx, a.tan_fovy, a.mh_dist, a.campos[0],
                                                      a.campos[1], a.campos[2], a.ntx, a.nty, o, a.table);
}

int launch_preprocess(const PreprocessArgs &a, hipStream_t st) {
  with_degree<0>(a.l_max, [&](auto L) {
    with_bool(a.store_mid, [&](auto mid) {
      with_bool(a.compact, [&](auto cmp) {
        with_bool(a.antialiased, [&](auto aa) {
          launch_per_gaussian(preprocess_kernel<decltype(L)::value, decltype(mid)::value, decltype(cmp)::value, decltype(aa)::value>, a, st);
        });
      });
    });
  });
  GS_LAUNCH_CHECK();
  return GSPLAT_OK;
}

int launch_preprocess_geom(const PreprocessArgs &a, int colour, hipStream_t st) {
  GS_REQUIRE(colour >= 0 && colour <= 2, "colour: 0 formed here, 1 read from rgb, 2 written by sh_colour_kernel");
  auto with_colour = [&](auto f) {
    if (colour == 0) f(std::integral_constant<int, 0>{});
    else if (colour == 1) f(std::integral_constant<int, 1>{});
    else f(std::integral_constant<int, 2>{});
  };
  with_colour([&](auto col) {
    with_bool(a.store_mid, [&](auto mid) {
      with_bool(a.compact, [&](auto cmp) {
        launch_per_gaussian(preprocess_geom_kernel<decltype(col)::value, decltype(mid)::value, decltype(cmp)::value>, a, st);
      });
    });
  });
  GS_LAUNCH_CHECK();
  return GSPLAT_OK;
}

int launch_sh_colour(const ShColourArgs &a, hipStream_t st) {
  GS_REQUIRE(a.l_max >= 1, "degree 0 has no colour kernel: preprocess_geom_kernel forms the colour itself");
  const dim3 grid(div_up(bin_chunks(a.g.num_gaussians), kBlock / 64)), block(kBlock);
  with_degree<1>(a.l_max, [&](auto L) {
    with_bool(a.compact, [&](auto cmp) {
      sh_colour_kernel<decltype(L)::value, decltype(cmp)::value><<<grid, block, 0, st>>>(
          a.g, a.mask, a.rank, a.chunk_first, a.slice_counts, a.kept, a.campos[0], a.campos[1], a.campos[2], a.rgb_out, a.recs);
    });
  });
  GS_LAUNCH_CHECK();
  return GSPLAT_OK;
}

size_t scan_counts_temp_bytes(size_t N) {
  size_t bytes = 0;
  (void)rocprim::exclusive_scan(nullptr, bytes, (int *)nullptr, (int *)nullptr, 0, N + 1, rocprim::plus<int>(), (hipStream_t)0);
  return bytes;
}

int launch_publish_counts(const int *rank_total, const int *offsets_total, const unsigned long long *pair_counters,
                          unsigned long long *pub, unsigned long long ticket, hipStream_t st) {
  publish_counts_kernel<<<1, 64, 0, st>>>(rank_total, offsets_total, pair_counters, pub, ticket);
  GS_LAUNCH_CHECK();
  return GSPLAT_OK;
}

}
```

3dgs_amd/csrc/gs_preprocess_bwd.hip:

```cpp
#include "gs_common.h"
#include "gs_launch.h"
#include "gs_math.h"
#include "gs_pergaussian_args.h"
#include "gs_render.h"
#include "gs_rows.h"

namespace {

constexpr int kBlock = 256;

struct BwdOut {
  float *xyz, *rgb, *sh, *opacity, *scale, *quaternion;
  float *conic, *uv, *J, *sigma, *xyz_c, *pre_rgb;
  float *common, *uv_norm;
};

__device__ __forceinline__ int first_slot_not_below(const int *__restrict__ c2g, int M, int key) {
  const int lane = threadIdx.x & 63;
  int lo = 0, hi = M;
  while (hi > lo) {
    const int step = (hi - lo + 63) >> 6;
    const long long p = (long long)lo + (long long)lane * step;
    const bool below = p < hi && c2g[p] < key;
    const int t = __popcll(__ballot(below));
    if (t == 0) {
      hi = lo;
    } else {
      const long long next = (long long)lo + (long long)t * step;
      hi = next < hi ? (int)next : hi;
      lo = lo + (t - 1) * step + 1;
    }
  }
  return lo;
}

struct AdamFused {
  float *m_xyz, *v_xyz, *m_rgb, *v_rgb, *m_sh, *v_sh, *m_op, *v_op, *m_sc, *v_sc, *m_q, *v_q;
  float lr_xyz, lr_rgb, lr_sh, lr_op, lr_sc, lr_q;
  float b1, b2, eps, bias1, bias2;
  float *uv_accum;
  int *accum_dur;
  float *dir;
};

#ifndef GS_BWD3_WAVES
#define GS_BWD3_WAVES 3
#endif
template <int L, int kAdam = 0, bool kDepthRow = false, bool kCamGrad = false, bool kAbsRow = false, bool kAntialias = false>
__global__ __launch_bounds__(kBlock) __attribute__((amdgpu_waves_per_eu(kAdam == 3 ? GS_BWD3_WAVES : 3, 8))) void preprocess_bwd_kernel(gsplat_gaussians g, const float *__restrict__ view,
                                                                const float *__restrict__ proj, int M,
                                                                const int *__restrict__ c2g,
                                                                const float *__restrict__ xyz_c_sel,
                                                                const float4 *__restrict__ rows_in, float fx, float fy,
                                                                float tan_fovx, float tan_fovy, float fwd_tan_fovx,
                                                                float fwd_tan_fovy, float mh_dist, float cx, float cy,
                                                                float cz, int width, int height, BwdOut o,
                                                                int ranged, int i_lo, int i_hi, AdamFused ad,
                                                                double *__restrict__ cam_rows) {
  static_assert(!kCamGrad || kAdam == 0, "the camera gradient is a form of the plain backward");
  static_assert(!(kCamGrad && kAbsRow), "the camera form stores no densification statistic");
  static_assert(!kAntialias || (kAdam == 0 && !kCamGrad), "anti-aliased mode is a form of the plain backward");
  int j_first = 0;
  if (ranged) {
    j_first = first_slot_not_below(c2g, M, i_lo);
    M = first_slot_not_below(c2g, M, i_hi);
  }
  const int j = j_first + blockIdx.x * kBlock + threadIdx.x;
  constexpr int n = (L + 1) * (L + 1), kRest = (n - 1) * 3;
  __shared__ __attribute__((aligned(16))) float s_sh[kRest > 0 && kAdam != 3 ? kBlock * kRest : 4];
  __shared__ float s_dir[kAdam == 2 && kRest > 0 ? kBlock * 7 : 1];
  const int lane = threadIdx.x & 63, wave_first = threadIdx.x - lane;
  const int jw = j_first + blockIdx.x * kBlock + wave_first;
  if (jw >= M) return;
  const int rows = min(64, M - jw);
  const bool live = j < M;
  const int i = c2g[live ? j : jw];
  float *wsh = s_sh + (kAdam != 3 ? wave_first * kRest : 0);
  if constexpr (kRest > 0 && kAdam != 3) {
    const int i0 = __builtin_amdgcn_readfirstlane(i);
    if (__all(!live || i == i0 + lane)) {
      gs::rows_to_lds<kRest>(g.sh + (size_t)i0 * kRest, wsh, rows, lane);
    } else {
      constexpr int kPieces = (kRest + 3) / 4, kPer = 64 / kPieces, kIter = (64 + kPer - 1) / kPer;
      static_assert(kPieces <= 64 && kPer >= 1, "row too long for one lane group");
      const int grp = lane / kPieces, piece = lane - grp * kPieces;
      const bool in_grp = grp < kPer;
      float4 v[kIter];
#pragma unroll
      for (int it = 0; it < kIter; ++it) {
        const int r = it * kPer + grp;
        const int ir = __shfl(i, r < rows ? r : 0, 64);
        v[it] = make_float4(0.0f, 0.0f, 0.0f, 0.0f);
        if (in_grp && r < rows) {
          const float *src = g.sh + (size_t)ir * kRest + 4 * piece;
          if (4 * piece + 3 < kRest) {
            v[it] = __builtin_bit_cast(float4, *reinterpret_cast<const gs::f4u *>(src));
          } else {
            v[it].x = src[0];
            if (4 * piece + 1 < kRest) v[it].y = src[1];
            if (4 * piece + 2 < kRest) v[it].z = src[2];
          }
        }
      }
#pragma unroll
      for (int it = 0; it < kIter; ++it) {
        const int r = it * kPer + grp;
        if (in_grp && r < rows) {
          float *dst = wsh + r * kRest + 4 * piece;
          dst[0] = v[it].x;
          if (4 * piece + 1 < kRest) dst[1] = v[it].y;
          if (4 * piece + 2 < kRest) dst[2] = v[it].z;
          if (4 * piece + 3 < kRest) dst[3] = v[it].w;
        }
      }
    }
    __builtin_amdgcn_fence(__ATOMIC_ACQ_REL, "wavefront");
    __builtin_amdgcn_wave_barrier();
  }
  if constexpr (kRest > 0 && kAdam == 2) {
    {
      const float4 ga = rows_in[4 * (live ? j : jw)];
      float ux, uy, uz, len;
      gs::view_dir(g.xyz[3 * i], g.xyz[3 * i + 1], g.xyz[3 * i + 2], cx, cy, cz, ux, uy, uz, len);
      float *d = s_dir + (wave_first + lane) * 7;
      d[0] = ux; d[1] = uy; d[2] = uz; d[3] = ga.x; d[4] = ga.y; d[5] = ga.z; d[6] = __int_as_float(i);
    }
    __builtin_amdgcn_fence(__ATOMIC_ACQ_REL, "wavefront");
    __builtin_amdgcn_wave_barrier();
    float *sh_p = const_cast<float *>(g.sh);
    const float *dirs = s_dir + wave_first * 7;
    constexpr int kPieces = (kRest + 3) / 4, kPer = 64 / kPieces, kIter = (64 + kPer - 1) / kPer, kAhead = 4;
// ... 17 lines not shown
            vq[u] = __builtin_bit_cast(float4, *reinterpret_cast<const gs::f4u *>(ad.v_sh + at[u]));
          } else {
            mq[u].x = ad.m_sh[at[u]]; vq[u].x = ad.v_sh[at[u]];
            if (nval > 1) { mq[u].y = ad.m_sh[at[u] + 1]; vq[u].y = ad.v_sh[at[u] + 1]; }
            if (nval > 2) { mq[u].z = ad.m_sh[at[u] + 2]; vq[u].z = ad.v_sh[at[u] + 2]; }
          }
        }
      }
#pragma unroll
      for (int u = 0; u < kAhead; ++u) {
        const int r = (it0 + u) * kPer + grp;
        if (it0 + u < kIter && in_grp && r < rows) {
          const float *d = dirs + r * 7;
          float Y[n];
          gs::sh_basis<L>(d[0], d[1], d[2], Y);
          const float *prow = wsh + r * kRest + 4 * piece;
          float pv[4] = {prow[0], nval > 1 ? prow[1] : 0.0f, nval > 2 ? prow[2] : 0.0f, nval > 3 ? prow[3] : 0.0f};
          float mv[4] = {mq[u].x, mq[u].y, mq[u].z, mq[u].w}, vv[4] = {vq[u].x, vq[u].y, vq[u].z, vq[u].w};
#pragma unroll
          for (int t = 0; t < 4; ++t) {
            if (t < nval) {
              const int c = 4 * piece + t, k = c / 3, ch = c - 3 * k;
              float yv = 0.0f;
#pragma unroll
              for (int q = 0; q < n - 1; ++q) yv = k == q ? Y[q + 1] : yv;
              const float grad = d[3 + ch] * yv;
              gs::adam_values(pv[t], mv[t], vv[t], grad, ad.lr_sh, ad.b1, ad.b2, ad.eps, ad.bias1, ad.bias2);
            }
          }
          if (nval == 4) {
            *reinterpret_cast<gs::f4u *>(sh_p + at[u]) = gs::f4u{pv[0], pv[1], pv[2], pv[3]};
            *reinterpret_cast<gs::f4u *>(ad.m_sh + at[u]) = gs::f4u{mv[0], mv[1], mv[2], mv[3]};
            *reinterpret_cast<gs::f4u *>(ad.v_sh + at[u]) = gs::f4u{vv[0], vv[1], vv[2], vv[3]};
          } else {
            for (int t = 0; t < nval; ++t) { sh_p[at[u] + t] = pv[t]; ad.m_sh[at[u] + t] = mv[t]; ad.v_sh[at[u] + t] = vv[t]; }
          }
        }
      }
    }
  }
  float gx = 0.0f, gy = 0.0f, gz = 0.0f, b0g[3] = {0.0f, 0.0f, 0.0f};
  const gs::Mat34 vw = gs::load_view(view);
  const gs::Mat44 pr = gs::load_proj(proj);
  const int jr = live ? j : jw;
  const float4 a = rows_in[4 * jr], b = rows_in[4 * jr + 1], c = rows_in[4 * jr + 2];
  const float g_rgb[3] = {a.x, a.y, a.z};
  const float g_op = a.w;
  const float g_con[3] = {b.x, b.y, b.z};
  const float g_u = b.w, g_v = c.x;
  const float n_u = kAbsRow ? c.z : g_u, n_v = kAbsRow ? c.w : g_v;
  if constexpr (kAdam == 3 && kRest > 0) {
    b0g[0] = g_rgb[0] * GS_SH_C0; b0g[1] = g_rgb[1] * GS_SH_C0; b0g[2] = g_rgb[2] * GS_SH_C0;
    gx = ad.dir[3 * (size_t)jr]; gy = ad.dir[3 * (size_t)jr + 1]; gz = ad.dir[3 * (size_t)jr + 2];
  } else {
    float *row = wsh + lane * kRest;
    gs::sh_bwd<L, kAdam == 0>(row, g.rgb + 3 * i, g.xyz[3 * i], g.xyz[3 * i + 1], g.xyz[3 * i + 2], cx, cy, cz, g_rgb, row, b0g,
                          gx, gy, gz);
  }
  if constexpr (kRest > 0 && kAdam == 0) {
    __builtin_amdgcn_fence(__ATOMIC_ACQ_REL, "wavefront");
    __builtin_amdgcn_wave_barrier();
    if (o.sh) gs::rows_from_lds<kRest>(o.sh + (size_t)jw * kRest, wsh, rows, lane);
  }
  if constexpr (!kCamGrad) {
    if (!live) return;
  }
  gx = 0.0f + gx; gy = 0.0f + gy; gz = 0.0f + gz;
  [[maybe_unused]] const float g_dir[3] = {gx, gy, gz};
  auto step3 = [&](const float *pc, float *m, float *v, const float *gr, float lr) {
    float *p = const_cast<float *>(pc);
#pragma unroll
    for (int k = 0; k < 3; ++k) {
      float pv = p[3 * i + k], mv = m[3 * i + k], vv = v[3 * i + k];
      gs::adam_values(pv, mv, vv, gr[k], lr, ad.b1, ad.b2, ad.eps, ad.bias1, ad.bias2);
      p[3 * i + k] = pv; m[3 * i + k] = mv; v[3 * i + k] = vv;
    }
  };
  if constexpr (kAdam != 0) {
    step3(g.rgb, ad.m_rgb, ad.v_rgb, b0g, ad.lr_rgb);
    {
      float pv = g.opacity[i], mv = ad.m_op[i], vv = ad.v_op[i];
      gs::adam_values(pv, mv, vv, g_op, ad.lr_op, ad.b1, ad.b2, ad.eps, ad.bias1, ad.bias2);
      const_cast<float *>(g.opacity)[i] = pv; ad.m_op[i] = mv; ad.v_op[i] = vv;
    }
    if (ad.uv_accum) ad.uv_accum[i] += sqrtf(n_u * n_u + n_v * n_v);
    if (ad.accum_dur) ad.accum_dur[i] += 1;
  }
  const int jc = kCamGrad ? jr : j;
  const float x = xyz_c_sel[3 * jc], y = xyz_c_sel[3 * jc + 1], z = xyz_c_sel[3 * jc + 2];
  float Jv[6], sg[6], con[3], rad_unused[4], dJ[6], dS[6];
  {
    const float4 q = reinterpret_cast<const float4 *>(g.quaternion)[i];
    const gs::RotScale rs = gs::rot_scale(q.x, q.y, q.z, q.w, g.scale[3 * i], g.scale[3 * i + 1], g.scale[3 * i + 2]);
    gs::sigma_from(rs, sg);
  }
  gs::jacobian(x, y, z, fx, fy, fwd_tan_fovx, fwd_tan_fovy, Jv);
  float dM[kCamGrad ? 6 : 1];
  [[maybe_unused]] float g_logit = g_op;
  if constexpr (kAntialias) {
    float rho, cov_raw[3], drho, dcov[3];
    gs::conic_radius<true>(Jv, sg, vw, mh_dist, con, rad_unused, &rho, cov_raw);
    gs::effective_opacity_bwd(g_op, gs::sigmoid_fast(g.opacity[i]), rho, g_logit, drho);
    gs::compensation_bwd(cov_raw, rho, drho, dcov);
    gs::conic_bwd<false, true>(Jv, sg, vw, con, g_con, dJ, dS, nullptr, dcov);
  } else {
    gs::conic_radius(Jv, sg, vw, mh_dist, con, rad_unused);
    gs::conic_bwd<kCamGrad>(Jv, sg, vw, con, g_con, dJ, dS, dM);
  }
#pragma unroll
  for (int k = 0; k < 6; ++k) { dJ[k] = 0.0f + dJ[k]; dS[k] = 0.0f + dS[k]; }
  [[maybe_unused]] float jt_dm[kCamGrad ? 9 : 1];
  if constexpr (kCamGrad) {
#pragma unroll
    for (int r = 0; r < 3; ++r)
#pragma unroll
      for (int k = 0; k < 3; ++k) jt_dm[3 * r + k] = Jv[r] * dM[k] + Jv[3 + r] * dM[3 + k];
  }
  float cxg, cyg, czg;
  gs::jacobian_bwd(x, y, z, fx, fy, tan_fovx, tan_fovy, dJ, cxg, cyg, czg);
  cxg = 0.0f + cxg; cyg = 0.0f + cyg; czg = 0.0f + czg;
  int i2 = i;
  asm volatile("" : "+v"(i2));
  const float4 q = reinterpret_cast<const float4 *>(g.quaternion)[i2];
  const gs::RotScale rs = gs::rot_scale(q.x, q.y, q.z, q.w, g.scale[3 * i2], g.scale[3 * i2 + 1], g.scale[3 * i2 + 2]);
  float dQ[4], dSc[3];
  gs::sigma_bwd(rs, dS, dQ, dSc);
  float px_, py_, pz_;
  gs::to_screen_bwd(pr, x, y, z, g_u, g_v, width, height, px_, py_, pz_);
  cxg += px_; cyg += py_; czg += pz_;
  if constexpr (kDepthRow) czg += c.y;
  float wx, wy, wz;
  gs::camera_space_bwd(vw, cxg, cyg, czg, wx, wy, wz);
  gx += wx; gy += wy; gz += wz;
  if constexpr (kAdam != 0) {
    if constexpr (kAdam == 2 || kAdam == 3) {
      const float gxyz[3] = {gx, gy, gz};
      step3(g.xyz, ad.m_xyz, ad.v_xyz, gxyz, ad.lr_xyz);
    }
    step3(g.scale, ad.m_sc, ad.v_sc, dSc, ad.lr_sc);
    {
      float4 pq = reinterpret_cast<const float4 *>(g.quaternion)[i];
      float4 mq = reinterpret_cast<const float4 *>(ad.m_q)[i], vq = reinterpret_cast<const float4 *>(ad.v_q)[i];
// ... 131 lines not shown
    dd[0] = k == q ? dY[q + 1][0] : dd[0]; dd[1] = k == q ? dY[q + 1][1] : dd[1]; dd[2] = k == q ? dY[q + 1][2] : dd[2];
  }
  const bool act = k < kCoef;
  const long long o = (row * kCoef + k) * 3;
  float p[3] = {0.0f, 0.0f, 0.0f};
  if (act) {
    float mm[3], vv[3];
#pragma unroll
    for (int c = 0; c < 3; ++c) { p[c] = sh[o + c]; mm[c] = m[o + c]; vv[c] = v[o + c]; }
    float pn[3] = {p[0], p[1], p[2]};
#pragma unroll
    for (int c = 0; c < 3; ++c) gs::adam_values(pn[c], mm[c], vv[c], gr[c] * yv, lr, b1, b2, eps, bias1, bias2);
#pragma unroll
    for (int c = 0; c < 3; ++c) { sh[o + c] = pn[c]; m[o + c] = mm[c]; v[o + c] = vv[c]; }
  }
  float x[3][3], acc[3][3];
#pragma unroll
  for (int a = 0; a < 3; ++a)
#pragma unroll
    for (int c = 0; c < 3; ++c) {
      const float leaf = dd[a] * p[c];
      float first = 0.0f;
      first += dY[0][a] * band0[3 * row + c];
      first += leaf;
      x[a][c] = acc[a][c] = k == 0 ? first : leaf;
    }
#pragma unroll
  for (int step = 1; step < kCoef; ++step)
#pragma unroll
    for (int a = 0; a < 3; ++a)
#pragma unroll
      for (int c = 0; c < 3; ++c)
        acc[a][c] = __int_as_float(__builtin_amdgcn_update_dpp(0, __float_as_int(acc[a][c]), 0x111 , 0xF, 0xF, true)) + x[a][c];
  if (k == kCoef - 1) {
    const float tx = gr[0] * acc[0][0] + gr[1] * acc[0][1] + gr[2] * acc[0][2];
    const float ty = gr[0] * acc[1][0] + gr[1] * acc[1][1] + gr[2] * acc[1][2];
    const float tz = gr[0] * acc[2][0] + gr[1] * acc[2][1] + gr[2] * acc[2][2];
    const float dot = tx * ux + ty * uy + tz * uz;
    dir_out[3 * (size_t)r] = (tx - dot * ux) / len;
    dir_out[3 * (size_t)r + 1] = (ty - dot * uy) / len;
    dir_out[3 * (size_t)r + 2] = (tz - dot * uz) / len;
  }
}

}

namespace gs {

int launch_preprocess_bwd(const PreprocessBwdArgs &a, hipStream_t st) {
  GS_REQUIRE(a.span > 0, "nothing to launch");
  GS_REQUIRE(a.adam_mode >= 0 && a.adam_mode <= 3 && (a.adam_mode == 0 || a.adam != nullptr), "bad Adam form");
  GS_REQUIRE(!a.cam_rows || (a.adam_mode == 0 && !a.antialiased), "the camera gradient is a form of the plain backward");
  GS_REQUIRE(!a.antialiased || a.adam_mode == 0, "anti-aliased mode is a form of the plain backward");
  const gsplat_gradients &g = a.out;
  const BwdOut o = {g.grad_xyz, g.grad_rgb, g.grad_sh, g.grad_opacity, g.grad_scale, g.grad_quaternion, g.grad_conic,
                    g.grad_uv, g.grad_J, g.grad_sigma, g.grad_xyz_c, g.grad_precompute_rgb, a.common, a.uv_norm};
  AdamFused ad = {};
  if (a.adam_mode) {
    const gsplat_adam_fused &p = *a.adam;
    ad = {p.exp_avg[0], p.exp_avg_sq[0], p.exp_avg[1], p.exp_avg_sq[1], p.exp_avg[2], p.exp_avg_sq[2],
          p.exp_avg[3], p.exp_avg_sq[3], p.exp_avg[4], p.exp_avg_sq[4], p.exp_avg[5], p.exp_avg_sq[5],
          p.lr[0], p.lr[1], p.lr[2], p.lr[3], p.lr[4], p.lr[5],
          p.b1, p.b2, p.eps, p.bias1, p.bias2, p.uv_grad_accum, p.grad_accum_dur, a.adam_dir};
  }
  const dim3 grid(div_up(a.span, kBlock)), block(kBlock);
  auto launch = [&](auto kernel) {
    kernel<<<grid, block, 0, st>>>(a.g, a.view, a.proj, a.M, a.c2g, a.xyz_c, a.rows, a.fx, a.fy, a.tan_fovx, a.tan_fovy,
                                   a.fwd_tan_fovx, a.fwd_tan_fovy, a.mh_dist, a.campos[0], a.campos[1], a.campos[2], a.width,
                                   a.height, o, a.ranged, a.first, a.end, ad, a.cam_rows);
  };
  with_degree<0>(a.l_max, [&](auto L) {
    with_bool(a.rows_depth, [&](auto dr) {
      constexpr int kL = decltype(L)::value;
      constexpr bool kDR = decltype(dr)::value;
      if (a.cam_rows) return launch(preprocess_bwd_kernel<kL, 0, kDR, true>);
      with_bool(a.rows_abs, [&](auto ab) {
        constexpr bool kAB = decltype(ab)::value;
        if (a.adam_mode == 1) launch(preprocess_bwd_kernel<kL, 1, kDR, false, kAB>);
        else if (a.adam_mode == 3) launch(preprocess_bwd_kernel<kL, 3, kDR, false, kAB>);
        else if (a.adam_mode) launch(preprocess_bwd_kernel<kL, 2, kDR, false, kAB>);
        else if (a.antialiased) launch(preprocess_bwd_kernel<kL, 0, kDR, false, kAB, true>);
        else launch(preprocess_bwd_kernel<kL, 0, kDR, false, kAB>);
      });
    });
  });
  GS_LAUNCH_CHECK();
  if (a.cam_rows) {
    cam_grad_finalize_kernel<<<1, kCamFinThreads, 0, st>>>(a.cam_rows, (int)div_up(a.span, 64), a.grad_view, a.grad_campos);
    GS_LAUNCH_CHECK();
  }
  return GSPLAT_OK;
}

int launch_sh_adam_dir(const ShAdamDirArgs &a, hipStream_t st) {
  GS_REQUIRE(a.l_max >= 1 && a.M > 0, "degree 0 has no SH group; nothing to launch for M = 0");
  const unsigned int blocks = (unsigned int)(((long long)a.M * 16 + kBlock - 1) / kBlock);
  with_degree<1>(a.l_max, [&](auto L) {
    sh_adam_dir_kernel<decltype(L)::value><<<blocks, kBlock, 0, st>>>(a.M, a.c2g, a.sh, a.m, a.v, a.lr, a.b1, a.b2, a.eps, a.bias1,
                                                                      a.bias2, a.xyz, a.band0, a.campos[0], a.campos[1],
                                                                      a.campos[2], a.rows, a.dir_out);
  });
  GS_LAUNCH_CHECK();
  return GSPLAT_OK;
}

}
```

3dgs_amd/raster.py:

```python
import ctypes

import numpy as np
import torch

from . import _lib
from ._lib import check


class _DevView:

    def __init__(self, ptr, shape, typestr, owner):
        self.__cuda_array_interface__ = {"shape": tuple(int(s) for s in shape), "typestr": typestr,
                                         "data": (int(ptr), False), "version": 2}
        self._owner = owner


def _view(ptr, shape, typestr, owner):
    if ptr is None and int(np.prod(shape)) != 0:
        return None
    if ptr is None or int(np.prod(shape)) == 0:
        dt = {"<f4": torch.float32, "<i4": torch.int32, "|u1": torch.uint8}[typestr]
        return torch.empty(tuple(shape), dtype=dt, device="cuda")
    return torch.as_tensor(_DevView(ptr, shape, typestr, owner), device="cuda")

# ... 166 lines not shown
            raise ValueError("%s must be a contiguous %s float32 device tensor" % (name, "[N,C]" if dims == 2 else "[H,W,C]"))
        return t

    def render_features(self, features, out=None):
        self._dense("features", features, 2)
        N, C = int(features.shape[0]), int(features.shape[1])
        if not 1 <= C <= 512:
            raise ValueError("features must have 1 .. 512 channels, not %d" % C)
        H, W = self._feature_map_shape()
        if out is None:
            out = torch.empty(H, W, C, dtype=torch.float32, device=features.device)
        elif tuple(self._dense("out", out, 3).shape) != (H, W, C):
            raise ValueError("out must be [%d,%d,%d], not %s" % (H, W, C, list(out.shape)))
        st = ctypes.c_void_p(torch.cuda.current_stream().cuda_stream)
        check(self._lib.gsplat_context_render_features(self._h, N, C, _ptr(features), _ptr(out), st))
        return out

    def lift_features(self, map, out):
        self._dense("map", map, 3)
        self._dense("out", out, 2)
        N, C = int(out.shape[0]), int(out.shape[1])
        if not 1 <= C <= 512:
            raise ValueError("out must have 1 .. 512 channels, not %d" % C)
        H, W = self._feature_map_shape()
        if tuple(map.shape) != (H, W, C):
            raise ValueError("map must be [%d,%d,%d], not %s" % (H, W, C, list(map.shape)))
        st = ctypes.c_void_p(torch.cuda.current_stream().cuda_stream)
        check(self._lib.gsplat_context_lift_features(self._h, N, C, _ptr(map), _ptr(out), st))
        return out

    def features_backward(self, features, grad_map):
        self._dense("features", features, 2)
        self._dense("grad_map", grad_map, 3)
        N, C = int(features.shape[0]), int(features.shape[1])
        if not 1 <= C <= 512:
            raise ValueError("features must have 1 .. 512 channels, not %d" % C)
        H, W = self._feature_map_shape()
        if tuple(grad_map.shape) != (H, W, C):
            raise ValueError("grad_map must be [%d,%d,%d], not %s" % (H, W, C, list(grad_map.shape)))
        st = ctypes.c_void_p(torch.cuda.current_stream().cuda_stream)
        check(self._lib.gsplat_context_features_backward(self._h, N, C, _ptr(features), _ptr(grad_map), st))

    def _feature_map_shape(self):
        if self._last_size is None:
            raise _lib.GsplatError(-3, "no forward pass recorded in this context")
        return self._last_size

    def set_preprocess_split(self, mode):
        check(self._lib.gsplat_context_set_preprocess_split(self._h, int(mode)))

    def set_compact_lists(self, enabled):
        check(self._lib.gsplat_context_set_compact_lists(self._h, int(bool(enabled))))

    def counters(self):
        v = (ctypes.c_longlong * 12)()
        self._lib.gsplat_context_get_counters(self._h, v, 12)
        return dict(forwards=int(v[0]), tail_redone=int(v[1]), compact_walks=int(v[2]), instance_growths=int(v[3]),
                    ordered_backwards=int(v[4]), segmented_backwards=int(v[5]), segmented_forwards=int(v[6]),
                    longest_chain=int(v[7]), chain_sum=int(v[8]), segment_fallbacks=int(v[9]),
                    compact_list_backwards=int(v[10]), useful_entries=int(v[11]))

    def set_timing(self, enabled, stages=None):
        if enabled and stages is not None:
            mask = 0
            for name in stages:
                mask |= 1 << self.STAGES.index(name)
            check(self._lib.gsplat_context_set_timing_stages(self._h, mask))
        else:
            check(self._lib.gsplat_context_set_timing(self._h, int(bool(enabled))))

    def get_timing(self):
        ms = (ctypes.c_double * 8)()
        cnt = (ctypes.c_longlong * 8)()
        self._lib.gsplat_context_get_timing(self._h, ms, cnt, 8)
        return {s: ((ms[i] / cnt[i]) if cnt[i] else 0.0, int(cnt[i])) for i, s in enumerate(self.STAGES)}

    @staticmethod
    def _structs(params, cam, l_max):
        g = _lib.Gaussians()
        g.num_gaussians = int(params["xyz"].shape[0])
        g.xyz, g.rgb, g.opacity = _ptr(params["xyz"]), _ptr(params["rgb"]), _ptr(params["opacity"])
        g.scale, g.quaternion = _ptr(params["scale"]), _ptr(params["quaternion"])
        g.sh = _ptr(params["sh"]) if l_max > 0 else None
        c = _lib.Camera()
        c.width, c.height = int(cam["width"]), int(cam["height"])
        c.focal_x, c.focal_y = float(cam["fx"]), float(cam["fy"])
        for k in range(3):
            c.campos[k] = float(cam["campos"][k])
        c.view, c.proj = _ptr(cam["view"]), _ptr(cam["proj"])
        return g, c

    def rasterize_image(self, params, cam, config, bg_color, l_max):
        g, c = self._structs(params, cam, l_max)
        if self._filter3d is not None and self._filter3d.numel() != g.num_gaussians:
            raise ValueError("the 3D filter has %d rows for %d gaussians" % (self._filter3d.numel(), g.num_gaussians))
        self._filter3d_fwd = self._filter3d
        if l_max > 0:
            want = ((l_max + 1) ** 2 - 1) * 3
            if params["sh"].numel() != g.num_gaussians * want:
                raise ValueError("sh must be packed at the current band's stride")
        cfg = _lib.RasterConfig(float(config["near_thresh"]), float(config["mh_dist"]), int(config["cull_mask_padding"]))
        fv = _lib.ForwardView()
        st = ctypes.c_void_p(torch.cuda.current_stream().cuda_stream)
        check(self._lib.gsplat_rasterize_image(self._h, ctypes.byref(g), ctypes.byref(c), ctypes.byref(cfg),
                                               float(bg_color), int(l_max), ctypes.byref(fv), st))
        N, M, S = g.num_gaussians, int(fv.num_culled), int(fv.num_splats)
        W, H = c.width, c.height
        T = ((W + 15) // 16) * ((H + 15) // 16)
        out = _LazyViews(
            dict(num_culled=M, num_pairs=int(fv.num_pairs), num_splats=S),
            dict(mask=(fv.mask, (N,), "|u1"), uv_all=(fv.uv, (N, 2), "<f4"), xyz_c_all=(fv.xyz_c, (N, 3), "<f4"),
                 compact_to_global=(fv.compact_to_global, (M,), "<i4"), sigma=(fv.sigma, (M, 6), "<f4"),
                 conic=(fv.conic, (M, 3), "<f4"), J=(fv.J, (M, 6), "<f4"), rgb=(fv.precomputed_rgb, (M, 3), "<f4"),
# ... 199 lines not shown
```

3dgs_amd/trainer.py:

```python
import math
import os

import numpy as np
import torch

from . import ops, raster
from .dist import TorchComm, ViewShardedStep
from .optimizer import B1, B2, EPS, AdamOptimizer, DEFAULT_LR
from .rows import MOMENT, PARAM, STAT, RowTable

DISTORTION_WEIGHT = 10.0
NORMAL_PRIOR_WEIGHT = 0.2
NORMAL_SMOOTH_WEIGHT = 0.2

DEFAULT_CONFIG = dict(
    DEFAULT_LR, near_thresh=0.3, mh_dist=3.0, cull_mask_padding=100, ssim_frac=0.2, use_background=True,
    use_background_end=2000, reset_opacity_interval=3000, reset_opacity_value=0.05, reset_opacity_start=1050,
    reset_opacity_end=5000, max_sh_band=3, add_sh_band_interval=1000, use_split=True, use_clone=True, use_delete=True,
    adaptive_control_start=500, adaptive_control_end=5000, adaptive_control_interval=100, max_gaussians=4250000,
    delete_opacity_threshold=0.02, uv_grad_threshold=0.0002, split_scale_factor=1.6,
    absgrad=False,
    antialiased=False,
    filter3d=False, filter3d_interval=100, filter3d_near=0.2,
    prune_contribution=False, prune_contribution_threshold=0.01, prune_contribution_interval=1000,
# ... 125 lines not shown
    def feature_channels(self):
        return int(self.cfg["features"])

    @property
    def num_gaussians(self):
        return int(self.params["xyz"].shape[0])

    def _rows(self):
        o = self.opt
        return RowTable(self.params, o.exp_avg, o.exp_avg_sq, o.uv_grad_accum, o.grad_accum_dur, self._feat)

    def _initial_features(self, features, n):
        C = self.feature_channels
        if not C:
            return None
        dev = self.params["xyz"].device
        if features is None:
            return torch.zeros(n, C, dtype=torch.float32, device=dev)
        if (not isinstance(features, torch.Tensor) or features.dtype != torch.float32 or features.device != dev
                or tuple(features.shape) != (n, C)):
            raise ValueError("features must be a float32 [%d,%d] tensor on %s: one row per gaussian, config key features "
                             "channels" % (n, C, dev))
        return features.contiguous()

    @property
    def features(self):
        return None if self._feat is None else self._feat[0]

    def _install(self, rows):
        rows.check()
        sh = rows.params["sh"]
        l_max = math.isqrt(sh.shape[1] + 1) - 1 if sh.dim() == 3 else -1
        if tuple(sh.shape[1:]) != ((l_max + 1) ** 2 - 1, 3):
            raise ValueError("sh is %s: not the coefficients of an SH degree" % (tuple(sh.shape),))
        if (rows.features is not None) != bool(self.feature_channels) or \
                (rows.features is not None and rows.features[0].shape[1] != self.feature_channels):
            raise ValueError("the table's feature column does not match config key features = %d" % self.feature_channels)
        self.l_max = l_max
        self._feat = rows.features
        if self._feat_grad is not None and self._feat_grad.shape[0] < rows.num_rows:
            self._feat_grad = None
        self.params = dict(rows.params)
        self.opt = AdamOptimizer({g: self.params[g] for g in rows.exp_avg}, self.l_max, lr_config=self.cfg,
                                 scene_extent=self.scene_extent,
                                 state=(rows.exp_avg, rows.exp_avg_sq, rows.uv_grad_accum, rows.grad_accum_dur))
        self._sharded = None
        self._filter3d = None

    def _new_context(self, n, W, H):
        ctx = raster.RasterContext(n, W, H)
        ctx.set_lean_forward(True)
        ctx.set_absgrad(bool(self.cfg["absgrad"]))
        ctx.set_antialiased(bool(self.cfg["antialiased"]))
        if self._depth_keys():
            ctx.set_depth(True, inverse=bool(self.cfg["distortion_inverse"]), moment=bool(self.cfg["distortion"]))
        return ctx

    def _context_for(self, n):
        if n > self.ctx_capacity:
            self.ctx_capacity = int(n * 1.5) + 1
            self.ctx = self._new_context(self.ctx_capacity, self.ctx.max_width, self.ctx.max_height)
        self._set_filter3d(self.ctx)
        return self.ctx

    @property
    def filter3d(self):
        if not self.cfg["filter3d"] or self.num_gaussians == 0:
            return None
        if self._filter3d is None:
            if self._filter3d_cams is None:
                self._filter3d_cams = ops.camera_arrays([v[0] for v in self.views], self.params["xyz"].device)
            self._filter3d = ops.compute_filter3d(self.params["xyz"], *self._filter3d_cams,
                                                  near=float(self.cfg["filter3d_near"]))
        return self._filter3d

    def _set_filter3d(self, ctx):
        if self.cfg["filter3d"] and ctx._filter3d is not self.filter3d:
            ctx.set_filter3d(self.filter3d)

    def _refresh_filter3d(self, it):
        if self.cfg["filter3d"] and it % int(self.cfg["filter3d_interval"]) == 0 and it > 0:
            self._filter3d = None

    def _grad_image_for(self, H, W, device):
        buf = self._grad_image.get((H, W))
        if buf is None:
            buf = self._grad_image[(H, W)] = torch.empty(H, W, 3, dtype=torch.float32, device=device)
        return buf

    def _gradients_for(self, ctx, m):
        n = self.num_gaussians
        if self._grads is None or self._grads[0] < n or self._grads[1] != self.l_max:
            self._grads = (n, self.l_max, ctx.alloc_gradients(n, self.l_max, intermediates=("uv",), factored_sh=True))
        return {k: (v[:m] if v is not None else None) for k, v in self._grads[2].items()}

    def _partial_gradients_for(self, ctx, m):
        n = self.num_gaussians
        if self._grads2 is None or self._grads2[0] < n:
            dev = self.params["xyz"].device
            self._grads2 = (n, dict(xyz=torch.empty(n, 3, device=dev), precompute_rgb=torch.empty(n, 3, device=dev)))
        return {k: v[:m] for k, v in self._grads2[1].items()}

    def _depth_keys(self):
        c = self.cfg
        return bool(c["distortion"] or c["depth_prior"] or c["normal_prior"] or c["normal_smooth"])

# ... 621 lines not shown
```

include/gsplat_hip.h:

```cpp
#ifndef GSPLAT_HIP_H
#define GSPLAT_HIP_H

#include <stddef.h>
#include <stdint.h>

#ifdef __cplusplus
extern "C" {
#endif

#define GSPLAT_OK 0
#define GSPLAT_ERR_NULL_POINTER (-1)
#define GSPLAT_ERR_NOT_DEVICE (-2)
#define GSPLAT_ERR_INVALID_ARG (-3)
#define GSPLAT_ERR_HIP (-4)
#define GSPLAT_ERR_NO_VISIBLE (-5)
#define GSPLAT_ERR_CAPACITY (-6)

#define GSPLAT_TILE_SIZE 16

const char *gsplat_last_error(void);
#define GSPLAT_ABI_VERSION 9
int gsplat_abi_version(void);
const char *gsplat_source_hash(void);
const char *gsplat_build_flags(void);
// ... 280 lines not shown

int gsplat_context_render_features(gsplat_context *ctx, int num_gaussians, int channels,
                                   const float *features , float *out ,
                                   void *stream);
int gsplat_context_lift_features(gsplat_context *ctx, int num_gaussians, int channels, const float *map ,
                                 float *lifted , void *stream);

int gsplat_context_features_backward(gsplat_context *ctx, int num_gaussians, int channels,
                                     const float *features ,
                                     const float *grad_map , void *stream);

int gsplat_feature_ce_loss(const float *map, const int *labels , int rows, int cols, int channels,
                           float weight, int accumulate, float *grad_map, float *loss_out, void *stream);
int gsplat_feature_l1_loss(const float *map, const float *target, const unsigned char *valid ,
                           int rows, int cols, int channels, float weight, int accumulate, float *grad_map,
                           float *loss_out, void *stream);
int gsplat_feature_cosine_loss(const float *map, const float *target, const unsigned char *valid ,
                               int rows, int cols, int channels, float weight, int accumulate, float *grad_map,
                               float *loss_out, void *stream);
int gsplat_feature_adam_step(const int *compact_to_global, int num_culled, int channels,
                             float *features, float *exp_avg, float *exp_avg_sq ,
                             float *grad_global , float lr, float b1, float b2,
                             float eps, float bias1, float bias2, void *stream);

int gsplat_bilagrid_slice(const float *grid, int grid_w, int grid_h, int grid_l, const float *image, int rows, int cols,
                          float *out, void *stream);
int gsplat_bilagrid_slice_backward(const float *grid, int grid_w, int grid_h, int grid_l, const float *image,
                                   const float *grad_out, int rows, int cols, int accumulate_grid,
                                   float *grad_image , float *grad_grid , void *stream);
int gsplat_bilagrid_tv_loss(const float *grid, int grid_w, int grid_h, int grid_l, float weight, int accumulate,
                            float *grad_grid, float *loss_out, void *stream);

int gsplat_vq_assign(const float *x, const float *codebook, int N, int D, int K, int *index, float *dist ,
                     void *stream);
int gsplat_vq_update(const float *x, const int *order, const int *start, int N, int D, int K, float *codebook,
                     void *stream);

int gsplat_context_set_binning_route(gsplat_context *ctx, int route);

int gsplat_context_set_segment_options(gsplat_context *ctx, int poll_budget, int thin_layer_blocks, float gate);

int gsplat_context_detach_forward_outputs(gsplat_context *ctx);
int gsplat_context_last_compaction(gsplat_context *ctx, const unsigned char **mask, const int **slots,
                                   const int **compact_to_global, int *num_gaussians, int *num_culled);
int gsplat_compact_rows_ranked(const float *src, const unsigned char *mask, const int *slots, int N, int stride,
                               float *dst, int dst_rows, void *stream);
int gsplat_fill_f32(float *dst, size_t n, float value, void *stream);
int gsplat_mask_selected_rows(const unsigned char *mask, int N, int *rows, int rows_cap, void *stream);
int gsplat_context_set_render_only(gsplat_context *ctx, int enabled);
int gsplat_context_set_lean_forward(gsplat_context *ctx, int enabled);
int gsplat_context_set_preprocess_split(gsplat_context *ctx, int mode);
int gsplat_context_get_counters(gsplat_context *ctx, long long *out, int n);
int gsplat_context_set_compact_lists(gsplat_context *ctx, int enabled);
int gsplat_context_set_timing(gsplat_context *ctx, int enabled);
int gsplat_context_set_timing_stages(gsplat_context *ctx, unsigned int stage_mask);
int gsplat_context_get_timing(gsplat_context *ctx, double *stage_ms_sum, long long *stage_count, int max_stages);

int gsplat_pack_gradients_global(gsplat_context *ctx, const gsplat_gradients *grads, int l_max, int num_gaussians,
                                 float *packed, void *stream);
int gsplat_packed_gradient_width(int l_max);

int gsplat_factored_gradient_width(int world_size);
int gsplat_pack_gradients_factored(gsplat_context *ctx, const gsplat_gradients *grads, int num_gaussians, int rank,
                                   int world_size, float *factored, void *stream);
int gsplat_unpack_gradients_factored(const float *xyz, const float *campos_all, const float *factored, int l_max,
                                     int num_gaussians, int world_size, float *packed, void *stream);


int gsplat_pack_gradients_split(gsplat_context *ctx, const gsplat_gradients *grads, int num_gaussians, float *common,
                                float *rgb, void *stream);
int gsplat_pack_gradients_split_range(gsplat_context *ctx, const gsplat_gradients *grads, int num_gaussians,
                                      int first_gaussian, int end_gaussian, float *common, float *rgb, void *stream);
int gsplat_unpack_gradients_split(const float *xyz, const float *common, const float *rgb_all, size_t rank_stride,
                                  int l_max, int num_gaussians, int world_size, float *packed, void *stream);

int gsplat_pack_uv_grad_norm(gsplat_context *ctx, const gsplat_gradients *grads, int num_gaussians, float *uv_norm,
                             void *stream);

int gsplat_context_set_absgrad(gsplat_context *ctx, int enabled);
int gsplat_context_absgrad_uv(gsplat_context *ctx, float *abs_uv, void *stream);
int gsplat_pack_absgrad_norm(gsplat_context *ctx, int num_gaussians, float *uv_norm, void *stream);

int gsplat_context_set_antialiased(gsplat_context *ctx, int enabled);
int gsplat_compute_conic_antialiased(const float *xyz, const float *view, const float *sigma, float focal_x,
                                     float focal_y, float tan_fovx, float tan_fovy, float mh_dist, int N, float *J,
                                     float *conic, float *radius, float *compensation, void *stream);
int gsplat_compute_conic_antialiased_backward(const float *J, const float *sigma, const float *view, const float *conic,
                                              const float *conic_grad_out, const float *compensation_grad_out, int N,
                                              float *J_grad_in, float *sigma_grad_in, void *stream);

int gsplat_compute_filter3d(const float *xyz, int N, const float *views, const float *projs, const float *focal_x,
                            const int *sizes, int V, float near_thresh, float *filter3d, void *stream);
int gsplat_filter3d_apply(const float *scale, const float *opacity, const float *filter3d, int N, float *scale_eff,
                          float *opacity_eff, void *stream);
int gsplat_filter3d_apply_backward(const float *scale, const float *opacity, const float *filter3d, const int *rows,
                                   int M, float *grad_scale, int scale_stride, float *grad_opacity, int opacity_stride,
                                   void *stream);
int gsplat_context_set_filter3d(gsplat_context *ctx, const float *filter3d);

#ifdef __cplusplus
}
#endif
#endif
```

Baseline: 1360 it/s.

## Cache SH direction-gradient sums from forward preprocess for reuse in backward

During forward preprocessing, the kernel now computes the nine per-Gaussian sums of SH basis gradients times SH coefficients and stores them in a per-context buffer, along with a ticket that records which inputs they came from. When the backward runs with the same inputs (plain or Adam mode 1, no camera gradient, no antialiasing), it reads these sums instead of reloading all SH coefficients into LDS and recomputing the basis gradients. It also recomputes camera-space position from xyz rather than reading it back. The cost is 36 bytes per Gaussian written in forward, extra work in the forward preprocess, and validity bookkeeping that falls back to the old path when anything changes.

```diff
diff --git a/3dgs_amd/_lib.py b/3dgs_amd/_lib.py
--- a/3dgs_amd/_lib.py
+++ b/3dgs_amd/_lib.py
@@ -230,6 +230,7 @@
     "gsplat_vq_update": (_I, [_P, _P, _P, _I, _I, _I, _P, _P]),
     "gsplat_context_set_absgrad": (_I, [_P, _I]),
     "gsplat_context_set_compact_lists": (_I, [_P, _I]),
+    "gsplat_context_set_dir_sums": (_I, [_P, _I]),
     "gsplat_context_absgrad_uv": (_I, [_P, _P, _P]),
     "gsplat_pack_absgrad_norm": (_I, [_P, _I, _P, _P]),
     "gsplat_context_set_antialiased": (_I, [_P, _I]),
diff --git a/3dgs_amd/csrc/gs_context.h b/3dgs_amd/csrc/gs_context.h
--- a/3dgs_amd/csrc/gs_context.h
+++ b/3dgs_amd/csrc/gs_context.h
@@ -11,6 +11,7 @@
 bool no_segments();
 bool no_fwd_segments();
 double fwd_segments_gate();
+bool no_dir_sums();
 
 }
 
@@ -69,6 +70,15 @@
   gs::DeviceBuffer kept;
   gs::DeviceBuffer dir_grad;
   gs::DeviceBuffer cam_rows;
+  gs::DeviceBuffer dir_sums;
+  bool dir_sums_on = true;
+  struct DirSumsOf {
+    unsigned long long ticket = 0;
+    const float *xyz = nullptr, *rgb = nullptr, *sh = nullptr, *view = nullptr;
+    float campos[3] = {0.f, 0.f, 0.f};
+  } dir_sums_of;
+  unsigned long long fwd_ticket = 0;
+  long long n_dir_sums_backwards = 0, n_dir_sums_fallbacks = 0;
   gs::SortFork fork;
   volatile unsigned long long *h_pub = nullptr;
   unsigned long long *d_pub = nullptr, ticket = 0;
@@ -116,7 +126,7 @@
     f(c.ids_c, W); f(c.masks_c, W); f(c.n_c_px, W); f(c.tile_useful, W);
     f(c.seg_first, W); f(c.seg_extra, W); f(c.seg_chk, W);
     f(c.fseg_first, W); f(c.fseg_blocks, W); f(c.fseg_gran, W); f(c.fseg_part, W); f(c.fseg_stop, W);
-    f(c.dir_grad, W); f(c.cam_rows, W); f(c.depth_map, W); f(c.seg_chk_d, W); f(c.fseg_part_d, W);
+    f(c.dir_grad, W); f(c.cam_rows, W); f(c.dir_sums, W); f(c.depth_map, W); f(c.seg_chk_d, W); f(c.fseg_part_d, W);
     f(c.depth2_map, W); f(c.seg_chk_q, W); f(c.fseg_part_q, W);
     f(c.f3d_scale, W); f(c.f3d_opacity, W);
     f(c.chunk_first, 0u);
diff --git a/3dgs_amd/csrc/gs_context.hip b/3dgs_amd/csrc/gs_context.hip
--- a/3dgs_amd/csrc/gs_context.hip
+++ b/3dgs_amd/csrc/gs_context.hip
@@ -21,6 +21,7 @@
 bool no_segments() { static const bool v = env_is("GSPLAT_NO_SEGMENTS", '1'); return v; }
 bool no_fwd_segments() { static const bool v = env_is("GSPLAT_NO_FWD_SEGMENTS", '1'); return v; }
 double fwd_segments_gate() { static const double v = env_number("GSPLAT_FWD_SEGMENTS_GATE", 3.0); return v; }
+bool no_dir_sums() { static const bool v = env_is("GSPLAT_NO_DIR_SUMS", '1'); return v; }
 
 size_t instance_room(const gsplat_context *c) {
   size_t room = c->keys_a.bytes / sizeof(unsigned int);
@@ -179,6 +180,12 @@
   return GSPLAT_OK;
 }
 
+int gsplat_context_set_dir_sums(gsplat_context *c, int enabled) {
+  GS_REQUIRE(c != nullptr, "null context");
+  c->dir_sums_on = enabled != 0;
+  return GSPLAT_OK;
+}
+
 int gsplat_context_set_absgrad(gsplat_context *c, int enabled) {
   GS_REQUIRE(c != nullptr, "null context");
   c->absgrad = enabled != 0;
@@ -307,11 +314,11 @@
     GS_HIP(hipMemcpy(h.data(), c->tile_useful.ptr, tiles * sizeof(int), hipMemcpyDeviceToHost));
     for (int u : h) useful += u;
   }
-  const long long v[12] = {c->n_forwards, c->n_tail_redone, c->n_compact_walks, c->n_instance_growths, c->n_ordered_backwards,
+  const long long v[14] = {c->n_forwards, c->n_tail_redone, c->n_compact_walks, c->n_instance_growths, c->n_ordered_backwards,
                            (long long)c->n_segmented_backwards, (long long)c->n_segmented_forwards, fmax, fsum, fallbacks,
-                           c->n_compact_backwards, useful};
-  for (int k = 0; k < n && k < 12; ++k) out[k] = v[k];
-  return 12;
+                           c->n_compact_backwards, useful, c->n_dir_sums_backwards, c->n_dir_sums_fallbacks};
+  for (int k = 0; k < n && k < 14; ++k) out[k] = v[k];
+  return 14;
 }
 
 int gsplat_context_set_render_only(gsplat_context *c, int enabled) {
diff --git a/3dgs_amd/csrc/gs_fused.hip b/3dgs_amd/csrc/gs_fused.hip
--- a/3dgs_amd/csrc/gs_fused.hip
+++ b/3dgs_amd/csrc/gs_fused.hip
@@ -15,6 +15,7 @@
   bool compact;
   bool beside;
   bool ro, mid;
+  bool sums;
   bool sparse, keys_ok;
   int *bin_table;
   unsigned long long ticket;
@@ -47,6 +48,7 @@
 static int reclaim_outputs(gsplat_context *c, hipStream_t st) {
   c->have_forward = c->lists_ready = c->rows_ready = c->order_ready = c->depth_ready = c->rows_depth = c->rows_abs = false;
   c->depth_inverse_ready = c->depth_moment_ready = false;
+  c->dir_sums_of.ticket = 0;
   gs::pool_unwatch(&c->last_mask);
   c->last_mask = nullptr;
   gs::DeviceBuffer *outs[13];
@@ -90,6 +92,8 @@
     }
   }
   f.ro = c->render_only; f.mid = !f.ro && !c->lean;
+  f.sums = c->dir_sums_on && !gs::no_dir_sums() && l_max > 0 && !f.ro && c->pre_split == 0 && !c->antialiased;
+  if (f.sums && (rc = c->dir_sums.reserve((size_t)c->max_gaussians * 9 * sizeof(float), st))) return rc;
   const bool want_dense = c->forced_route == 2 || (c->forced_route == 0 && c->dense_route);
   f.sparse = !want_dense && gs::binning_supports_counting_sort(f.num_tiles);
   if (f.sparse) {
@@ -172,8 +176,15 @@
       if (gs::pre_join_late()) f.join_pending = true;
       else GS_HIP(hipStreamWaitEvent(st, c->ev_pre_join, 0));
     }
-  } else if ((rc = gs::launch_preprocess(a, st))) {
-    return rc;
+  } else {
+    if (f.sums) a.dir_sums = c->dir_sums.as<float>();
+    if ((rc = gs::launch_preprocess(a, st))) return rc;
+    if (f.sums) {
+      gsplat_context::DirSumsOf &of = c->dir_sums_of;
+      of.ticket = f.ticket;
+      of.xyz = f.g->xyz; of.rgb = f.g->rgb; of.sh = f.g->sh; of.view = f.cam->view;
+      for (int k = 0; k < 3; ++k) of.campos[k] = f.cam->campos[k];
+    }
   }
   c->fwd_antialiased = c->antialiased;
   return GSPLAT_OK;
@@ -405,6 +416,7 @@
   gs::pool_watch(c->last_mask, &c->last_mask);
   c->tan_fovx = f.tan_fovx; c->tan_fovy = f.tan_fovy; c->mh_dist = f.cfg->mh_dist;
   c->have_forward = !f.ro;
+  c->fwd_ticket = f.ticket;
   c->lists_ready = true;
   c->depth_ready = c->depth;
   c->depth_inverse_ready = c->depth && f.dmap.inverse;
@@ -465,6 +477,7 @@
     if ((rc = finish_radix_route(c, f, rec, room))) return rc;
   } else if (gs::tail_needs_redo(rec.S, room, spec_hint, rec.longest, f.keys_ok)) {
     c->n_tail_redone++;
+    c->dir_sums_of.ticket = 0;
     if (rec.S > room) {
       c->n_instance_growths++;
       if ((rc = gs::reserve_instances(c, rec.S + rec.S / 4, f.num_tiles, st))) return rc;
@@ -667,6 +680,16 @@
   if (cam_grad) { a.cam_rows = c->cam_rows.as<double>(); a.grad_view = grad_view; a.grad_campos = grad_campos; }
   a.l_max = l_max; a.rows_depth = c->rows_depth; a.rows_abs = c->rows_abs;
   a.antialiased = c->fwd_antialiased;
+  {
+    const gsplat_context::DirSumsOf &of = c->dir_sums_of;
+    const bool sums = c->dir_sums_on && !gs::no_dir_sums() && (!adam || adam_mode == 1) && !cam_grad && !a.antialiased && c->dir_sums.ptr != nullptr && of.ticket != 0 &&
+                      of.ticket == c->fwd_ticket && of.xyz == g->xyz && of.rgb == g->rgb &&
+                      of.sh == g->sh && of.view == cam->view && of.campos[0] == cam->campos[0] && of.campos[1] == cam->campos[1] &&
+                      of.campos[2] == cam->campos[2];
+    if (sums) a.dir_sums = c->dir_sums.as<float>();
+    (sums ? c->n_dir_sums_backwards : c->n_dir_sums_fallbacks)++;
+    if (adam) c->dir_sums_of.ticket = 0;
+  }
   if ((rc = gs::launch_preprocess_bwd(a, st))) return rc;
   if (c->fwd_filter3d) {
     const int lo = whole ? 0 : first_gaussian, hi = whole ? 0 : end_gaussian;
diff --git a/3dgs_amd/csrc/gs_math.h b/3dgs_amd/csrc/gs_math.h
--- a/3dgs_amd/csrc/gs_math.h
+++ b/3dgs_amd/csrc/gs_math.h
@@ -162,59 +162,74 @@
 #define GS_SH_C8 0.3731763325901154f
 #define GS_SH_C9 1.445305721320277f
 
+template <int B>
+__device__ __forceinline__ void sh_basis_band(float x, float y, float z, float *Y) {
+  static_assert(B >= 0 && B <= 3, "bands 0..3");
+  if constexpr (B == 0) {
+    Y[0] = GS_SH_C0;
+  } else if constexpr (B == 1) {
+    Y[0] = GS_SH_C1 * y; Y[1] = GS_SH_C1 * z; Y[2] = GS_SH_C1 * x;
+  } else if constexpr (B == 2) {
+    const float xx = x * x, yy = y * y, zz = z * z;
+    Y[0] = GS_SH_C2 * (x * y);
+    Y[1] = GS_SH_C2 * (y * z);
+    Y[2] = GS_SH_C3 * (2.0f * zz - xx - yy);
+    Y[3] = GS_SH_C2 * (x * z);
+    Y[4] = GS_SH_C4 * (xx - yy);
+  } else {
+    const float xx = x * x, yy = y * y, zz = z * z;
+    Y[0] = GS_SH_C5 * (y * (3.0f * xx - yy));
+    Y[1] = GS_SH_C6 * (x * y * z);
+    Y[2] = GS_SH_C7 * (y * (4.0f * zz - xx - yy));
+    Y[3] = GS_SH_C8 * (z * (2.0f * zz - 3.0f * xx - 3.0f * yy));
+    Y[4] = GS_SH_C7 * (x * (4.0f * zz - xx - yy));
+    Y[5] = GS_SH_C9 * (z * (xx - yy));
+    Y[6] = GS_SH_C5 * (x * (xx - 3.0f * yy));
+  }
+}
 template <int L>
 __device__ __forceinline__ void sh_basis(float x, float y, float z, float *Y) {
-  Y[0] = GS_SH_C0;
-  if constexpr (L >= 1) {
-    Y[1] = GS_SH_C1 * y; Y[2] = GS_SH_C1 * z; Y[3] = GS_SH_C1 * x;
-  }
-  if constexpr (L >= 2) {
+  sh_basis_band<0>(x, y, z, Y);
+  if constexpr (L >= 1) sh_basis_band<1>(x, y, z, Y + 1);
+  if constexpr (L >= 2) sh_basis_band<2>(x, y, z, Y + 4);
+  if constexpr (L >= 3) sh_basis_band<3>(x, y, z, Y + 9);
+}
+
+template <int B>
+__device__ __forceinline__ void sh_basis_grad_band(float x, float y, float z, float (*d)[3]) {
+  static_assert(B >= 0 && B <= 3, "bands 0..3");
+  if constexpr (B == 0) {
+    d[0][0] = d[0][1] = d[0][2] = 0.0f;
+  } else if constexpr (B == 1) {
+    d[0][0] = 0; d[0][1] = GS_SH_C1; d[0][2] = 0;
+    d[1][0] = 0; d[1][1] = 0; d[1][2] = GS_SH_C1;
+    d[2][0] = GS_SH_C1; d[2][1] = 0; d[2][2] = 0;
+  } else if constexpr (B == 2) {
+    d[0][0] = GS_SH_C2 * y; d[0][1] = GS_SH_C2 * x; d[0][2] = 0;
+    d[1][0] = 0; d[1][1] = GS_SH_C2 * z; d[1][2] = GS_SH_C2 * y;
+    d[2][0] = GS_SH_C3 * (-2.0f * x); d[2][1] = GS_SH_C3 * (-2.0f * y); d[2][2] = GS_SH_C3 * (4.0f * z);
+    d[3][0] = GS_SH_C2 * z; d[3][1] = 0; d[3][2] = GS_SH_C2 * x;
+    d[4][0] = GS_SH_C4 * (2.0f * x); d[4][1] = GS_SH_C4 * (-2.0f * y); d[4][2] = 0;
+  } else {
     const float xx = x * x, yy = y * y, zz = z * z;
-    Y[4] = GS_SH_C2 * (x * y);
-    Y[5] = GS_SH_C2 * (y * z);
-    Y[6] = GS_SH_C3 * (2.0f * zz - xx - yy);
-    Y[7] = GS_SH_C2 * (x * z);
-    Y[8] = GS_SH_C4 * (xx - yy);
-    if constexpr (L >= 3) {
-      Y[9] = GS_SH_C5 * (y * (3.0f * xx - yy));
-      Y[10] = GS_SH_C6 * (x * y * z);
-      Y[11] = GS_SH_C7 * (y * (4.0f * zz - xx - yy));
-      Y[12] = GS_SH_C8 * (z * (2.0f * zz - 3.0f * xx - 3.0f * yy));
-      Y[13] = GS_SH_C7 * (x * (4.0f * zz - xx - yy));
-      Y[14] = GS_SH_C9 * (z * (xx - yy));
-      Y[15] = GS_SH_C5 * (x * (xx - 3.0f * yy));
-    }
-  }
-}
-
+    d[0][0] = GS_SH_C5 * (6.0f * x * y); d[0][1] = GS_SH_C5 * (3.0f * xx - 3.0f * yy); d[0][2] = 0;
+    d[1][0] = GS_SH_C6 * (y * z); d[1][1] = GS_SH_C6 * (x * z); d[1][2] = GS_SH_C6 * (x * y);
+    d[2][0] = GS_SH_C7 * (-2.0f * x * y); d[2][1] = GS_SH_C7 * (4.0f * zz - xx - 3.0f * yy);
+    d[2][2] = GS_SH_C7 * (8.0f * y * z);
+    d[3][0] = GS_SH_C8 * (-6.0f * x * z); d[3][1] = GS_SH_C8 * (-6.0f * y * z);
+    d[3][2] = GS_SH_C8 * (6.0f * zz - 3.0f * xx - 3.0f * yy);
+    d[4][0] = GS_SH_C7 * (4.0f * zz - 3.0f * xx - yy); d[4][1] = GS_SH_C7 * (-2.0f * x * y);
+    d[4][2] = GS_SH_C7 * (8.0f * x * z);
+    d[5][0] = GS_SH_C9 * (2.0f * x * z); d[5][1] = GS_SH_C9 * (-2.0f * y * z); d[5][2] = GS_SH_C9 * (xx - yy);
+    d[6][0] = GS_SH_C5 * (3.0f * xx - 3.0f * yy); d[6][1] = GS_SH_C5 * (-6.0f * x * y); d[6][2] = 0;
+  }
+}
 template <int L>
 __device__ __forceinline__ void sh_basis_grad(float x, float y, float z, float (*d)[3]) {
-  d[0][0] = d[0][1] = d[0][2] = 0.0f;
-  if constexpr (L >= 1) {
-    d[1][0] = 0; d[1][1] = GS_SH_C1; d[1][2] = 0;
-    d[2][0] = 0; d[2][1] = 0; d[2][2] = GS_SH_C1;
-    d[3][0] = GS_SH_C1; d[3][1] = 0; d[3][2] = 0;
-  }
-  if constexpr (L >= 2) {
-    const float xx = x * x, yy = y * y, zz = z * z;
-    d[4][0] = GS_SH_C2 * y; d[4][1] = GS_SH_C2 * x; d[4][2] = 0;
-    d[5][0] = 0; d[5][1] = GS_SH_C2 * z; d[5][2] = GS_SH_C2 * y;
-    d[6][0] = GS_SH_C3 * (-2.0f * x); d[6][1] = GS_SH_C3 * (-2.0f * y); d[6][2] = GS_SH_C3 * (4.0f * z);
-    d[7][0] = GS_SH_C2 * z; d[7][1] = 0; d[7][2] = GS_SH_C2 * x;
-    d[8][0] = GS_SH_C4 * (2.0f * x); d[8][1] = GS_SH_C4 * (-2.0f * y); d[8][2] = 0;
-    if constexpr (L >= 3) {
-      d[9][0] = GS_SH_C5 * (6.0f * x * y); d[9][1] = GS_SH_C5 * (3.0f * xx - 3.0f * yy); d[9][2] = 0;
-      d[10][0] = GS_SH_C6 * (y * z); d[10][1] = GS_SH_C6 * (x * z); d[10][2] = GS_SH_C6 * (x * y);
-      d[11][0] = GS_SH_C7 * (-2.0f * x * y); d[11][1] = GS_SH_C7 * (4.0f * zz - xx - 3.0f * yy);
-      d[11][2] = GS_SH_C7 * (8.0f * y * z);
-      d[12][0] = GS_SH_C8 * (-6.0f * x * z); d[12][1] = GS_SH_C8 * (-6.0f * y * z);
-      d[12][2] = GS_SH_C8 * (6.0f * zz - 3.0f * xx - 3.0f * yy);
-      d[13][0] = GS_SH_C7 * (4.0f * zz - 3.0f * xx - yy); d[13][1] = GS_SH_C7 * (-2.0f * x * y);
-      d[13][2] = GS_SH_C7 * (8.0f * x * z);
-      d[14][0] = GS_SH_C9 * (2.0f * x * z); d[14][1] = GS_SH_C9 * (-2.0f * y * z); d[14][2] = GS_SH_C9 * (xx - yy);
-      d[15][0] = GS_SH_C5 * (3.0f * xx - 3.0f * yy); d[15][1] = GS_SH_C5 * (-6.0f * x * y); d[15][2] = 0;
-    }
-  }
+  sh_basis_grad_band<0>(x, y, z, d);
+  if constexpr (L >= 1) sh_basis_grad_band<1>(x, y, z, d + 1);
+  if constexpr (L >= 2) sh_basis_grad_band<2>(x, y, z, d + 4);
+  if constexpr (L >= 3) sh_basis_grad_band<3>(x, y, z, d + 9);
 }
 
 __device__ __forceinline__ void view_dir(float px, float py, float pz, float cx, float cy, float cz, float &dx,
@@ -503,6 +518,97 @@
   dQ[3] = rs.inv_norm * (dz - dot * z);
 }
 
+template <int B, class F>
+__device__ __forceinline__ void sh_dir_sums_band(const float *sh, float ux, float uy, float uz, float *s , F &&each_k) {
+  constexpr int k0 = B * B - 1, nb = 2 * B + 1;
+  float d[nb][3];
+#pragma unroll
+  for (int m = 0; m < nb; ++m) {
+    const int k = k0 + m;
+    const float Ri = sh[3 * k], Gi = sh[3 * k + 1], Bi = sh[3 * k + 2];
+    each_k(k, ux, uy, uz, s);
+    if (m == 0) sh_basis_grad_band<B>(ux, uy, uz, d);
+    const float ddx = d[m][0], ddy = d[m][1], ddz = d[m][2];
+    s[0] += ddx * Ri; s[1] += ddx * Gi; s[2] += ddx * Bi;
+    s[3] += ddy * Ri; s[4] += ddy * Gi; s[5] += ddy * Bi;
+    s[6] += ddz * Ri; s[7] += ddz * Gi; s[8] += ddz * Bi;
+  }
+}
+template <int L, bool kLazy = false, class F>
+__device__ __forceinline__ void sh_dir_sums(const float *sh, const float *__restrict__ band0, float ux, float uy, float uz,
+                                            float *s , F &&each_k) {
+  constexpr int n = (L + 1) * (L + 1);
+  if constexpr (kLazy) {
+#pragma unroll
+    for (int k = 0; k < 9; ++k) s[k] = 0;
+    {
+      float d0[1][3];
+      sh_basis_grad_band<0>(ux, uy, uz, d0);
+      const float R0 = band0[0], G0 = band0[1], B0 = band0[2];
+      s[0] += d0[0][0] * R0; s[1] += d0[0][0] * G0; s[2] += d0[0][0] * B0;
+      s[3] += d0[0][1] * R0; s[4] += d0[0][1] * G0; s[5] += d0[0][1] * B0;
+      s[6] += d0[0][2] * R0; s[7] += d0[0][2] * G0; s[8] += d0[0][2] * B0;
+    }
+    if constexpr (L >= 1) sh_dir_sums_band<1>(sh, ux, uy, uz, s, each_k);
+    if constexpr (L >= 2) sh_dir_sums_band<2>(sh, ux, uy, uz, s, each_k);
+    if constexpr (L >= 3) sh_dir_sums_band<3>(sh, ux, uy, uz, s, each_k);
+  } else {
+    float dY[n][3];
+    sh_basis_grad<L>(ux, uy, uz, dY);
+    float dRx = 0, dGx = 0, dBx = 0, dRy = 0, dGy = 0, dBy = 0, dRz = 0, dGz = 0, dBz = 0;
+    {
+      const float R0 = band0[0], G0 = band0[1], B0 = band0[2];
+      dRx += dY[0][0] * R0; dGx += dY[0][0] * G0; dBx += dY[0][0] * B0;
+      dRy += dY[0][1] * R0; dGy += dY[0][1] * G0; dBy += dY[0][1] * B0;
+      dRz += dY[0][2] * R0; dGz += dY[0][2] * G0; dBz += dY[0][2] * B0;
+    }
+#pragma unroll
+    for (int k = 0; k < n - 1; ++k) {
+      const float Ri = sh[3 * k], Gi = sh[3 * k + 1], Bi = sh[3 * k + 2];
+      each_k(k);
+      const float ddx = dY[k + 1][0], ddy = dY[k + 1][1], ddz = dY[k + 1][2];
+      dRx += ddx * Ri; dGx += ddx * Gi; dBx += ddx * Bi;
+      dRy += ddy * Ri; dGy += ddy * Gi; dBy += ddy * Bi;
+      dRz += ddz * Ri; dGz += ddz * Gi; dBz += ddz * Bi;
+    }
+    s[0] = dRx; s[1] = dGx; s[2] = dBx; s[3] = dRy; s[4] = dGy; s[5] = dBy; s[6] = dRz; s[7] = dGz; s[8] = dBz;
+  }
+}
+template <int L>
+__device__ __forceinline__ void sh_dir_sums(const float *sh, const float *__restrict__ band0, float ux, float uy, float uz,
+                                            float *s ) {
+  sh_dir_sums<L>(sh, band0, ux, uy, uz, s, [](int) {});
+}
+
+template <int L, class F>
+__device__ __forceinline__ void sh_to_rgb_dir_sums(const float *sh, const float *__restrict__ band0, float dx, float dy,
+                                                   float dz, float *rgb, float *s , F &&pin) {
+  float Y[16];
+  sh_basis_band<0>(dx, dy, dz, Y);
+  float r = band0[0] * Y[0] + 0.5f, g = band0[1] * Y[0] + 0.5f, b = band0[2] * Y[0] + 0.5f;
+  sh_dir_sums<L, true>(sh, band0, dx, dy, dz, s, [&](int k, float &x, float &y, float &z, float *acc) {
+    if (k == 0 || k == 3 || k == 5 || k == 8 || k == 11) pin(x, y, z, acc, r, g, b);
+    if (k == 0) sh_basis_band<1>(x, y, z, Y + 1);
+    if (k == 3) sh_basis_band<2>(x, y, z, Y + 4);
+    if (k == 8) sh_basis_band<3>(x, y, z, Y + 9);
+    r += sh[3 * k + 0] * Y[k + 1];
+    g += sh[3 * k + 1] * Y[k + 1];
+    b += sh[3 * k + 2] * Y[k + 1];
+  });
+  rgb[0] = r; rgb[1] = g; rgb[2] = b;
+}
+
+__device__ __forceinline__ void sh_dir_finish(const float *s , const float *gr, float ux, float uy, float uz, float len,
+                                              float &ox, float &oy, float &oz) {
+  const float tx = gr[0] * s[0] + gr[1] * s[1] + gr[2] * s[2];
+  const float ty = gr[0] * s[3] + gr[1] * s[4] + gr[2] * s[5];
+  const float tz = gr[0] * s[6] + gr[1] * s[7] + gr[2] * s[8];
+  const float dot = tx * ux + ty * uy + tz * uz;
+  ox = (tx - dot * ux) / len;
+  oy = (ty - dot * uy) / len;
+  oz = (tz - dot * uz) / len;
+}
+
 template <int L, bool kStoreGrad = true>
 __device__ __forceinline__ void sh_bwd(const float *sh, const float *__restrict__ band0, float px,
                                        float py, float pz, float cx, float cy, float cz, const float *gr,
@@ -512,34 +618,14 @@
   float ux, uy, uz, len;
   view_dir(px, py, pz, cx, cy, cz, ux, uy, uz, len);
   float Y[n];
-  float dY[n][3];
   sh_basis<L>(ux, uy, uz, Y);
-  sh_basis_grad<L>(ux, uy, uz, dY);
   band0_grad[0] = gr[0] * Y[0]; band0_grad[1] = gr[1] * Y[0]; band0_grad[2] = gr[2] * Y[0];
-  float dRx = 0, dGx = 0, dBx = 0, dRy = 0, dGy = 0, dBy = 0, dRz = 0, dGz = 0, dBz = 0;
-  {
-    const float R0 = band0[0], G0 = band0[1], B0 = band0[2];
-    dRx += dY[0][0] * R0; dGx += dY[0][0] * G0; dBx += dY[0][0] * B0;
-    dRy += dY[0][1] * R0; dGy += dY[0][1] * G0; dBy += dY[0][1] * B0;
-    dRz += dY[0][2] * R0; dGz += dY[0][2] * G0; dBz += dY[0][2] * B0;
-  }
-#pragma unroll
-  for (int k = 0; k < n - 1; ++k) {
+  float s[9];
+  sh_dir_sums<L>(sh, band0, ux, uy, uz, s, [&](int k) {
     const float yv = Y[k + 1];
-    const float Ri = sh[3 * k], Gi = sh[3 * k + 1], Bi = sh[3 * k + 2];
     if constexpr (kStoreGrad) { sh_grad[3 * k] = gr[0] * yv; sh_grad[3 * k + 1] = gr[1] * yv; sh_grad[3 * k + 2] = gr[2] * yv; }
-    const float ddx = dY[k + 1][0], ddy = dY[k + 1][1], ddz = dY[k + 1][2];
-    dRx += ddx * Ri; dGx += ddx * Gi; dBx += ddx * Bi;
-    dRy += ddy * Ri; dGy += ddy * Gi; dBy += ddy * Bi;
-    dRz += ddz * Ri; dGz += ddz * Gi; dBz += ddz * Bi;
-  }
-  const float tx = gr[0] * dRx + gr[1] * dGx + gr[2] * dBx;
-  const float ty = gr[0] * dRy + gr[1] * dGy + gr[2] * dBy;
-  const float tz = gr[0] * dRz + gr[1] * dGz + gr[2] * dBz;
-  const float dot = tx * ux + ty * uy + tz * uz;
-  ox = (tx - dot * ux) / len;
-  oy = (ty - dot * uy) / len;
-  oz = (tz - dot * uz) / len;
+  });
+  sh_dir_finish(s, gr, ux, uy, uz, len, ox, oy, oz);
 }
 
 __device__ __forceinline__ void adam_values(float &p, float &m, float &v, float g, float lr, float b1, float b2, float eps,
diff --git a/3dgs_amd/csrc/gs_pergaussian_args.h b/3dgs_amd/csrc/gs_pergaussian_args.h
--- a/3dgs_amd/csrc/gs_pergaussian_args.h
+++ b/3dgs_amd/csrc/gs_pergaussian_args.h
@@ -30,6 +30,7 @@
   int *counts;
   unsigned long long *hitmask, *pairs;
   int *table;
+  float *dir_sums;
   int l_max;
   bool store_mid;
   bool compact;
@@ -64,6 +65,7 @@
   float *adam_dir;
   double *cam_rows;
   float *grad_view, *grad_campos;
+  const float *dir_sums;
   int l_max;
   int adam_mode;
   bool rows_depth, rows_abs, antialiased;
diff --git a/3dgs_amd/csrc/gs_preprocess.hip b/3dgs_amd/csrc/gs_preprocess.hip
--- a/3dgs_amd/csrc/gs_preprocess.hip
+++ b/3dgs_amd/csrc/gs_preprocess.hip
@@ -103,9 +103,10 @@
   int *counts;
   unsigned long long *hitmask;
   unsigned long long *pairs;
+  float *dir_sums;
 };
 
-template <int L, bool kStoreMid, bool kCompact, bool kAntialias = false>
+template <int L, bool kStoreMid, bool kCompact, bool kAntialias = false, bool kDirSums = false>
 __global__ __launch_bounds__(gs::kBinThreads) void preprocess_kernel(gsplat_gaussians g, const float *__restrict__ view,
                                                             const unsigned char *__restrict__ mask,
                                                             int *__restrict__ rank,
@@ -182,7 +183,26 @@
     const gs::Mat34 vw = gs::load_view(view);
     float dx, dy, dz, len, rgb[3];
     gs::view_dir(g.xyz[3 * i], g.xyz[3 * i + 1], g.xyz[3 * i + 2], cx, cy, cz, dx, dy, dz, len);
-    gs::sh_to_rgb<L>(g.sh + (size_t)i * (n - 1) * 3, g.rgb + 3 * i, dx, dy, dz, rgb);
+    if constexpr (kDirSums) {
+      constexpr int kRow = (n - 1) * 3;
+      float row[kRow > 0 ? kRow : 1], b0[3];
+      {
+        const float *src = g.sh + (size_t)i * kRow;
+#pragma unroll
+        for (int k = 0; k < kRow; ++k) row[k] = src[k];
+        b0[0] = g.rgb[3 * i]; b0[1] = g.rgb[3 * i + 1]; b0[2] = g.rgb[3 * i + 2];
+      }
+      float ds[9];
+      gs::sh_to_rgb_dir_sums<L>(row, b0, dx, dy, dz, rgb, ds, [](float &x, float &y, float &z, float *s, float &r, float &g, float &b) {
+        asm volatile("" : "+v"(x), "+v"(y), "+v"(z), "+v"(s[0]), "+v"(s[1]), "+v"(s[2]), "+v"(s[3]), "+v"(s[4]), "+v"(s[5]),
+                          "+v"(s[6]), "+v"(s[7]), "+v"(s[8]), "+v"(r), "+v"(g), "+v"(b));
+      });
+      float *dst = o.dir_sums + 9 * (size_t)j;
+#pragma unroll
+      for (int k = 0; k < 9; ++k) dst[k] = ds[k];
+    } else {
+      gs::sh_to_rgb<L>(g.sh + (size_t)i * (n - 1) * 3, g.rgb + 3 * i, dx, dy, dz, rgb);
+    }
     const float4 q = reinterpret_cast<const float4 *>(g.quaternion)[i];
     const gs::RotScale rs = gs::rot_scale(q.x, q.y, q.z, q.w, g.scale[3 * i], g.scale[3 * i + 1], g.scale[3 * i + 2]);
     float sg[6], J[6], con[3], rad[4];
@@ -651,7 +671,8 @@
 
 template <class Kernel>
 static void launch_per_gaussian(Kernel kernel, const PreprocessArgs &a, hipStream_t st) {
-  const PreOut o = {a.c2g, a.xyz_c, a.uv, a.sigma, a.conic, a.J, a.rgb, a.radius, a.recs, a.counts, a.hitmask, a.pairs};
+  const PreOut o = {a.c2g, a.xyz_c, a.uv, a.sigma, a.conic, a.J, a.rgb, a.radius, a.recs, a.counts, a.hitmask, a.pairs,
+                    a.dir_sums};
   const size_t hist_bytes = a.table ? (size_t)a.ntx * a.nty * sizeof(int) : 0;
   kernel<<<kBinBlocks, kBinThreads, hist_bytes, st>>>(a.g, a.view, a.mask, a.rank, a.slice_counts, a.kept, a.proj, a.width,
                                                       a.height, a.fx, a.fy, a.tan_fovx, a.tan_fovy, a.mh_dist, a.campos[0],
@@ -659,12 +680,15 @@
 }
 
 int launch_preprocess(const PreprocessArgs &a, hipStream_t st) {
+  GS_REQUIRE(!(a.antialiased && a.dir_sums), "the anti-aliased forward has no form that writes the direction sums");
   with_degree<0>(a.l_max, [&](auto L) {
     with_bool(a.store_mid, [&](auto mid) {
       with_bool(a.compact, [&](auto cmp) {
-        with_bool(a.antialiased, [&](auto aa) {
-          launch_per_gaussian(preprocess_kernel<decltype(L)::value, decltype(mid)::value, decltype(cmp)::value, decltype(aa)::value>, a, st);
-        });
+        constexpr int kL = decltype(L)::value;
+        constexpr bool kMid = decltype(mid)::value, kCmp = decltype(cmp)::value;
+        if (a.antialiased) launch_per_gaussian(preprocess_kernel<kL, kMid, kCmp, true>, a, st);
+        else if (a.dir_sums) launch_per_gaussian(preprocess_kernel<kL, kMid, kCmp, false, true>, a, st);
+        else launch_per_gaussian(preprocess_kernel<kL, kMid, kCmp, false>, a, st);
       });
     });
   });
diff --git a/3dgs_amd/csrc/gs_preprocess_bwd.hip b/3dgs_amd/csrc/gs_preprocess_bwd.hip
--- a/3dgs_amd/csrc/gs_preprocess_bwd.hip
+++ b/3dgs_amd/csrc/gs_preprocess_bwd.hip
@@ -46,7 +46,8 @@
 #ifndef GS_BWD3_WAVES
 #define GS_BWD3_WAVES 3
 #endif
-template <int L, int kAdam = 0, bool kDepthRow = false, bool kCamGrad = false, bool kAbsRow = false, bool kAntialias = false>
+template <int L, int kAdam = 0, bool kDepthRow = false, bool kCamGrad = false, bool kAbsRow = false, bool kAntialias = false,
+          bool kDirSums = false>
 __global__ __launch_bounds__(kBlock) __attribute__((amdgpu_waves_per_eu(kAdam == 3 ? GS_BWD3_WAVES : 3, 8))) void preprocess_bwd_kernel(gsplat_gaussians g, const float *__restrict__ view,
                                                                 const float *__restrict__ proj, int M,
                                                                 const int *__restrict__ c2g,
@@ -56,7 +57,10 @@
                                                                 float fwd_tan_fovy, float mh_dist, float cx, float cy,
                                                                 float cz, int width, int height, BwdOut o,
                                                                 int ranged, int i_lo, int i_hi, AdamFused ad,
-                                                                double *__restrict__ cam_rows) {
+                                                                double *__restrict__ cam_rows,
+                                                                const float *__restrict__ dir_sums) {
+  static_assert(!kDirSums || ((kAdam == 0 || kAdam == 1) && !kCamGrad && !kAntialias),
+                "the direction sums are read by the plain form and by kAdam 1 only");
   static_assert(!kCamGrad || kAdam == 0, "the camera gradient is a form of the plain backward");
   static_assert(!(kCamGrad && kAbsRow), "the camera form stores no densification statistic");
   static_assert(!kAntialias || (kAdam == 0 && !kCamGrad), "anti-aliased mode is a form of the plain backward");
@@ -67,7 +71,7 @@
   }
   const int j = j_first + blockIdx.x * kBlock + threadIdx.x;
   constexpr int n = (L + 1) * (L + 1), kRest = (n - 1) * 3;
-  __shared__ __attribute__((aligned(16))) float s_sh[kRest > 0 && kAdam != 3 ? kBlock * kRest : 4];
+  __shared__ __attribute__((aligned(16))) float s_sh[kRest > 0 && kAdam != 3 && !(kDirSums && kAdam != 0) ? kBlock * kRest : 4];
   __shared__ float s_dir[kAdam == 2 && kRest > 0 ? kBlock * 7 : 1];
   const int lane = threadIdx.x & 63, wave_first = threadIdx.x - lane;
   const int jw = j_first + blockIdx.x * kBlock + wave_first;
@@ -75,8 +79,8 @@
   const int rows = min(64, M - jw);
   const bool live = j < M;
   const int i = c2g[live ? j : jw];
-  float *wsh = s_sh + (kAdam != 3 ? wave_first * kRest : 0);
-  if constexpr (kRest > 0 && kAdam != 3) {
+  float *wsh = s_sh + (kAdam != 3 && !(kDirSums && kAdam != 0) ? wave_first * kRest : 0);
+  if constexpr (kRest > 0 && kAdam != 3 && !kDirSums) {
     const int i0 = __builtin_amdgcn_readfirstlane(i);
     if (__all(!live || i == i0 + lane)) {
       gs::rows_to_lds<kRest>(g.sh + (size_t)i0 * kRest, wsh, rows, lane);
@@ -200,6 +204,24 @@
   if constexpr (kAdam == 3 && kRest > 0) {
     b0g[0] = g_rgb[0] * GS_SH_C0; b0g[1] = g_rgb[1] * GS_SH_C0; b0g[2] = g_rgb[2] * GS_SH_C0;
     gx = ad.dir[3 * (size_t)jr]; gy = ad.dir[3 * (size_t)jr + 1]; gz = ad.dir[3 * (size_t)jr + 2];
+  } else if constexpr (kDirSums) {
+    float s[9];
+#pragma unroll
+    for (int k = 0; k < 9; ++k) s[k] = dir_sums[9 * (size_t)jr + k];
+    float ux, uy, uz, len;
+    gs::view_dir(g.xyz[3 * i], g.xyz[3 * i + 1], g.xyz[3 * i + 2], cx, cy, cz, ux, uy, uz, len);
+    float Y[n];
+    gs::sh_basis<L>(ux, uy, uz, Y);
+    b0g[0] = g_rgb[0] * Y[0]; b0g[1] = g_rgb[1] * Y[0]; b0g[2] = g_rgb[2] * Y[0];
+    if constexpr (kAdam == 0) {
+      [[maybe_unused]] float *row = wsh + lane * kRest;
+#pragma unroll
+      for (int k = 0; k < n - 1; ++k) {
+        const float yv = Y[k + 1];
+        row[3 * k] = g_rgb[0] * yv; row[3 * k + 1] = g_rgb[1] * yv; row[3 * k + 2] = g_rgb[2] * yv;
+      }
+    }
+    gs::sh_dir_finish(s, g_rgb, ux, uy, uz, len, gx, gy, gz);
   } else {
     float *row = wsh + lane * kRest;
     gs::sh_bwd<L, kAdam == 0>(row, g.rgb + 3 * i, g.xyz[3 * i], g.xyz[3 * i + 1], g.xyz[3 * i + 2], cx, cy, cz, g_rgb, row, b0g,
@@ -235,7 +257,12 @@
     if (ad.accum_dur) ad.accum_dur[i] += 1;
   }
   const int jc = kCamGrad ? jr : j;
-  const float x = xyz_c_sel[3 * jc], y = xyz_c_sel[3 * jc + 1], z = xyz_c_sel[3 * jc + 2];
+  float x, y, z;
+  if constexpr (kDirSums) {
+    gs::camera_space(vw, g.xyz[3 * i], g.xyz[3 * i + 1], g.xyz[3 * i + 2], x, y, z);
+  } else {
+    x = xyz_c_sel[3 * jc]; y = xyz_c_sel[3 * jc + 1]; z = xyz_c_sel[3 * jc + 2];
+  }
   float Jv[6], sg[6], con[3], rad_unused[4], dJ[6], dS[6];
   {
     const float4 q = reinterpret_cast<const float4 *>(g.quaternion)[i];
@@ -473,6 +500,8 @@
   GS_REQUIRE(a.adam_mode >= 0 && a.adam_mode <= 3 && (a.adam_mode == 0 || a.adam != nullptr), "bad Adam form");
   GS_REQUIRE(!a.cam_rows || (a.adam_mode == 0 && !a.antialiased), "the camera gradient is a form of the plain backward");
   GS_REQUIRE(!a.antialiased || a.adam_mode == 0, "anti-aliased mode is a form of the plain backward");
+  GS_REQUIRE(!a.dir_sums || (a.adam_mode <= 1 && !a.cam_rows && !a.antialiased),
+             "the direction sums are read by the plain form and by adam_mode 1 only");
   const gsplat_gradients &g = a.out;
   const BwdOut o = {g.grad_xyz, g.grad_rgb, g.grad_sh, g.grad_opacity, g.grad_scale, g.grad_quaternion, g.grad_conic,
                     g.grad_uv, g.grad_J, g.grad_sigma, g.grad_xyz_c, g.grad_precompute_rgb, a.common, a.uv_norm};
@@ -488,7 +517,7 @@
   auto launch = [&](auto kernel) {
     kernel<<<grid, block, 0, st>>>(a.g, a.view, a.proj, a.M, a.c2g, a.xyz_c, a.rows, a.fx, a.fy, a.tan_fovx, a.tan_fovy,
                                    a.fwd_tan_fovx, a.fwd_tan_fovy, a.mh_dist, a.campos[0], a.campos[1], a.campos[2], a.width,
-                                   a.height, o, a.ranged, a.first, a.end, ad, a.cam_rows);
+                                   a.height, o, a.ranged, a.first, a.end, ad, a.cam_rows, a.dir_sums);
   };
   with_degree<0>(a.l_max, [&](auto L) {
     with_bool(a.rows_depth, [&](auto dr) {
@@ -497,10 +526,12 @@
       if (a.cam_rows) return launch(preprocess_bwd_kernel<kL, 0, kDR, true>);
       with_bool(a.rows_abs, [&](auto ab) {
         constexpr bool kAB = decltype(ab)::value;
-        if (a.adam_mode == 1) launch(preprocess_bwd_kernel<kL, 1, kDR, false, kAB>);
+        if (a.adam_mode == 1 && a.dir_sums) launch(preprocess_bwd_kernel<kL, 1, kDR, false, kAB, false, true>);
+        else if (a.adam_mode == 1) launch(preprocess_bwd_kernel<kL, 1, kDR, false, kAB>);
         else if (a.adam_mode == 3) launch(preprocess_bwd_kernel<kL, 3, kDR, false, kAB>);
         else if (a.adam_mode) launch(preprocess_bwd_kernel<kL, 2, kDR, false, kAB>);
         else if (a.antialiased) launch(preprocess_bwd_kernel<kL, 0, kDR, false, kAB, true>);
+        else if (a.dir_sums) launch(preprocess_bwd_kernel<kL, 0, kDR, false, kAB, false, true>);
         else launch(preprocess_bwd_kernel<kL, 0, kDR, false, kAB>);
       });
     });
diff --git a/3dgs_amd/raster.py b/3dgs_amd/raster.py
--- a/3dgs_amd/raster.py
+++ b/3dgs_amd/raster.py
@@ -242,13 +242,17 @@
     def set_compact_lists(self, enabled):
         check(self._lib.gsplat_context_set_compact_lists(self._h, int(bool(enabled))))
 
+    def set_dir_sums(self, enabled):
+        check(self._lib.gsplat_context_set_dir_sums(self._h, int(bool(enabled))))
+
     def counters(self):
-        v = (ctypes.c_longlong * 12)()
-        self._lib.gsplat_context_get_counters(self._h, v, 12)
+        v = (ctypes.c_longlong * 14)()
+        self._lib.gsplat_context_get_counters(self._h, v, 14)
         return dict(forwards=int(v[0]), tail_redone=int(v[1]), compact_walks=int(v[2]), instance_growths=int(v[3]),
                     ordered_backwards=int(v[4]), segmented_backwards=int(v[5]), segmented_forwards=int(v[6]),
                     longest_chain=int(v[7]), chain_sum=int(v[8]), segment_fallbacks=int(v[9]),
-                    compact_list_backwards=int(v[10]), useful_entries=int(v[11]))
+                    compact_list_backwards=int(v[10]), useful_entries=int(v[11]),
+                    dir_sums_backwards=int(v[12]), dir_sums_fallbacks=int(v[13]))
 
     def set_timing(self, enabled, stages=None):
         if enabled and stages is not None:
diff --git a/3dgs_amd/trainer.py b/3dgs_amd/trainer.py
--- a/3dgs_amd/trainer.py
+++ b/3dgs_amd/trainer.py
@@ -201,6 +201,7 @@
         ctx.set_lean_forward(True)
         ctx.set_absgrad(bool(self.cfg["absgrad"]))
         ctx.set_antialiased(bool(self.cfg["antialiased"]))
+        ctx.set_dir_sums(self.fused_adam in (0, 1))
         if self._depth_keys():
             ctx.set_depth(True, inverse=bool(self.cfg["distortion_inverse"]), moment=bool(self.cfg["distortion"]))
         return ctx
diff --git a/include/gsplat_hip.h b/include/gsplat_hip.h
--- a/include/gsplat_hip.h
+++ b/include/gsplat_hip.h
@@ -356,6 +356,7 @@
 int gsplat_context_set_preprocess_split(gsplat_context *ctx, int mode);
 int gsplat_context_get_counters(gsplat_context *ctx, long long *out, int n);
 int gsplat_context_set_compact_lists(gsplat_context *ctx, int enabled);
+int gsplat_context_set_dir_sums(gsplat_context *ctx, int enabled);
 int gsplat_context_set_timing(gsplat_context *ctx, int enabled);
 int gsplat_context_set_timing_stages(gsplat_context *ctx, unsigned int stage_mask);
 int gsplat_context_get_timing(gsplat_context *ctx, double *stage_ms_sum, long long *stage_count, int max_stages);
```

After: 1396 it/s, median of 6. 1.03x the previous value.
